# paulvoliva/XNODE-WAN-PDE-solver

Measured on AMD Instinct MI355X. Metric: WAN training-steps/sec (optimiser sub-steps, d=20 cube, N_r=4096 paths per GPU), higher is better.
Workload: dtype f64

## Files before the change

xnode_wan_pde_solver_amd/_lib.py:

```python
import ctypes
import os

_HERE = os.path.dirname(os.path.abspath(__file__))
LIB_PATH = os.environ.get('XW_LIBRARY') or os.path.join(_HERE, 'libxnwan.so')
ABI_VERSION = 33

c_f32p = ctypes.c_void_p
c_f64p = ctypes.c_void_p
c_i64p = ctypes.c_void_p
c_int, c_dbl, c_vp = ctypes.c_int, ctypes.c_double, ctypes.c_void_p


class XwOdeFwdJob(ctypes.Structure):
    _fields_ = [('xT', c_vp), ('start', c_vp), ('u', c_vp), ('Y', c_vp), ('act', c_vp), ('N', c_int), ('act_x_only', c_int),
                ('narrow', c_int), ('prio_drop', c_int)]


class XwOdeBwdJob(ctypes.Structure):
    _fields_ = [('xT', c_vp), ('start', c_vp), ('Y', c_vp), ('act', c_vp), ('ubar', c_vp), ('gx', c_vp), ('gs', c_vp),
                ('gslab', c_vp), ('N', c_int), ('res_first_only', c_int), ('res_u', c_vp), ('res_ref', c_vp),
                ('res_coef', ctypes.c_double), ('res_base', ctypes.c_double), ('res_w_per_point', c_int), ('res_w', c_vp),
                ('res_c', c_vp), ('res_cp', c_vp), ('res_kappa2', ctypes.c_double), ('res_scal', c_vp), ('res_refA', c_vp),
                ('res_coefA', ctypes.c_double), ('res_baseA', ctypes.c_double)]

# ... 52 lines not shown
    'xw_ode_act_rows': [c_int, c_int, c_int, c_int],
    'xw_ode_bwd_multi': [ctypes.POINTER(XwOdeBwdJob), c_int, c_f32p, c_f64p, c_int, c_int, c_int, c_int, c_int, c_int, c_int, c_vp],
    'xw_tiled_ode_ok': [c_int, c_int, c_int, c_int],
    'xw_tiled_ode_work': [c_int, c_int, c_int, c_int, c_int],
    'xw_tiled_ode_bwd_slabs': [c_int],
    'xw_tiled_ode_fwd_multi': [ctypes.POINTER(XwOdeFwdJob), c_int, c_f32p, c_f64p, c_int, c_int, c_int, c_int, c_int, c_int, c_f64p,
                               c_f64p, c_vp],
    'xw_tiled_ode_bwd_multi': [ctypes.POINTER(XwOdeBwdJob), c_int, c_f32p, c_f64p, c_int, c_int, c_int, c_int, c_int, c_int, c_int,
                               c_f64p, c_vp],
    'xw_paths_tiled_work': [c_int, c_int, c_int, c_int],
    'xw_paths_tiled_fwd': [ctypes.POINTER(XwPathsJob), c_int, c_f64p, c_int, c_int, c_int, c_int, c_int, c_int, c_f64p, c_vp],
    'xw_adams_coef': [c_int, c_vp],
    'xw_adams_tiled_work': [c_int, c_int, c_int, c_int, c_int],
    'xw_adams_tiled_fwd_multi': [ctypes.POINTER(XwOdeFwdJob), c_int, c_f32p, c_f64p, c_int, c_int, c_int, c_int, c_int, c_f64p, c_f64p,
                                 c_vp],
    'xw_adams_tiled_bwd_multi': [ctypes.POINTER(XwOdeBwdJob), c_int, c_f32p, c_f64p, c_int, c_int, c_int, c_int, c_int, c_int, c_f64p,
                                 c_vp],
    'xw_dopri5_ctl_size': [],
    'xw_dopri5_work_size': [c_int],
    'xw_dopri5_init': [ctypes.POINTER(XwDopriJob), c_int, c_f32p, c_f64p, c_int, c_int, c_int, c_int, c_int, c_int, c_dbl, c_dbl,
                       c_vp],
    'xw_dopri5_attempts': [ctypes.POINTER(XwDopriJob), c_int, c_f32p, c_f64p, c_int, c_int, c_int, c_int, c_int, c_int, c_dbl,
                           c_dbl, c_int, c_int, c_vp],
    'xw_dopri5_sweep': [ctypes.POINTER(XwDopriSweepJob), c_int, c_f32p, c_f64p, c_int, c_int, c_int, c_int, c_int, c_int, c_vp],
    'xw_tdopri5_work': [c_int, c_int, c_int, c_int, c_int],
    'xw_tdopri5_part_size': [c_int],
    'xw_tdopri5_init': [ctypes.POINTER(XwDopriJob), c_int, c_f32p, c_f64p, c_int, c_int, c_int, c_int, c_int, c_int, c_dbl, c_dbl,
                        c_f64p, c_vp],
    'xw_tdopri5_attempts': [ctypes.POINTER(XwDopriJob), c_int, c_f32p, c_f64p, c_int, c_int, c_int, c_int, c_int, c_int, c_dbl,
                            c_dbl, c_int, c_int, c_f64p, c_vp],
    'xw_tdopri5_sweep': [ctypes.POINTER(XwDopriSweepJob), c_int, c_f32p, c_f64p, c_int, c_int, c_int, c_int, c_int, c_int, c_f64p,
                         c_vp],
    'xw_ode_bwd': [c_f32p, c_f32p, c_f64p, c_f64p, c_f64p, c_f64p, c_int, c_int, c_int, c_int, c_int, c_int, c_int, c_int,
                   c_f64p, c_f64p, c_f64p, c_vp],
    'xw_disc_fwd': [c_f32p, c_f32p, c_f32p, c_f64p, c_int, c_int, c_int, c_int, c_int, c_f64p, c_f64p, c_f64p, c_f64p, c_int,
                    c_int, c_f64p, c_vp],
    'xw_disc_xproj': [c_f32p, c_f64p, c_int, c_int, c_int, c_f64p, c_vp],
    'xw_disc_fwd_xproj': [c_f32p, c_f32p, c_f32p, c_f64p, c_int, c_int, c_int, c_int, c_int, c_f64p, c_f64p, c_f64p, c_f64p, c_int,
                          c_int, c_f64p, c_f64p, c_vp],
    'xw_disc_act_rows': [c_int, c_int],
    'xw_disc_gradx': [c_f32p, c_f32p, c_f32p, c_f64p, c_f64p, c_int, c_int, c_int, c_int, c_f64p, c_f64p, c_vp],
    'xw_disc_bwd_slabs': [c_int, c_int],
    'xw_disc_bwd': [c_f32p, c_f32p, c_f32p, c_f64p, c_f64p, c_int, c_int, c_int, c_int, c_int, c_f64p, c_f64p, c_vp],
    'xw_disc_tiled_ok': [c_int, c_int, c_int],
    'xw_disc_tiled_act_rows': [c_int, c_int],
    'xw_disc_tiled_fwd': [c_f32p, c_f32p, c_f32p, c_f64p, c_int, c_int, c_int, c_int, c_int, c_f64p, c_f64p, c_f64p, c_f64p, c_int,
                          c_int, c_f64p, c_f64p, c_vp],
    'xw_disc_tiled_bwd': [c_f32p, c_f32p, c_f32p, c_f64p, c_f64p, c_int, c_int, c_int, c_int, c_int, c_f64p, c_f64p, c_vp],
    'xw_mt19937_uniform_f32': [c_vp, ctypes.c_long, c_vp, ctypes.c_long, ctypes.c_float, ctypes.c_float, c_int],
    'xw_gather_fields': [c_vp, c_int, ctypes.c_long, c_vp],
    'xw_mt19937_legacy_normal_f64': [c_vp, ctypes.POINTER(c_int), ctypes.POINTER(c_int), ctypes.POINTER(c_dbl), c_vp, ctypes.c_long],
    'xw_weak_partials': [c_f64p, c_f64p, c_f64p, c_f64p, c_int, c_f64p, c_f64p, c_f64p, c_f64p, c_f64p, c_f64p, c_f64p,
                         c_f64p, c_int, c_f64p, c_dbl, c_f64p, c_f64p, c_f64p, c_int, c_dbl, c_int, c_int, c_dbl, c_dbl, c_f64p, c_f64p,
                         c_int, c_int, c_dbl, c_dbl, c_dbl, c_dbl, c_i64p, c_f64p, c_f64p, ctypes.c_long, c_vp],
    'xw_pair_fold': [c_f64p, c_dbl, c_dbl, c_vp],
    'xw_cube_weight': [c_vp, c_int, c_int, c_dbl, c_dbl, c_f64p, c_f64p, c_f64p, c_f64p, c_vp],
    'xw_bdry_partials': [c_f64p, c_f64p, c_int, c_int, c_dbl, c_dbl, c_f64p, c_f64p, c_f64p, c_vp],
    'xw_reduce_work_size': [],
    'xw_weak_contract_general': [c_f64p, c_int, c_f64p, c_f64p, c_f64p, c_f64p, c_f64p, c_f64p, c_f64p, c_f64p, c_int, c_int, c_f64p, c_vp],
    'xw_gen_cotangents': [c_f64p, c_f64p, c_f64p, c_int, c_f64p, c_f64p, c_dbl, c_f64p, c_int, c_int, c_dbl, c_dbl, c_dbl,
                          c_dbl, c_f64p, c_f64p, c_f64p, c_vp],
    'xw_disc_cotangent': [c_f64p, c_f64p, c_f64p, c_int, c_f64p, c_dbl, c_f64p, c_f64p, c_int, c_int, c_dbl, c_dbl, c_dbl,
                          c_dbl, c_f64p, c_f64p, c_vp],
    'xw_losses': [c_f64p, c_int, c_int, c_dbl, c_dbl, c_dbl, c_dbl, c_dbl, c_dbl, c_i64p, c_vp],
    'xw_adam': [c_f64p, c_f64p, c_int, c_f64p, c_f64p, c_int, c_f64p, c_f64p, c_f64p, c_f64p, c_i64p, c_int, c_int, c_dbl,
                c_dbl, c_dbl, c_dbl, c_f64p, c_int, c_int, c_int, c_i64p, c_vp],
    'xw_substep_gen': [ctypes.POINTER(XwGroup), ctypes.POINTER(XwSolverState), c_int, c_int, c_f64p, c_int, c_vp],
    'xw_substep_disc': [ctypes.POINTER(XwGroup), ctypes.POINTER(XwSolverState), c_int, c_int, c_f64p, c_vp],
    'xw_slab_sum': [c_f64p, c_int, c_int, c_int, c_f64p, c_vp],
    'xw_slab_sum2': [c_f64p, c_int, c_f64p, c_f64p, c_int, c_f64p, c_int, c_vp],
    'xw_comm_available': [],
    'xw_comm_unique_id': [ctypes.c_char_p],
    'xw_comm_init': [ctypes.c_char_p, c_int, c_int, ctypes.POINTER(c_vp)],
    'xw_allreduce': [c_f64p, c_int, c_vp, c_vp],
    'xw_comm_destroy': [c_vp],
}

EVAL_SIGNATURES = {
    'xw_paths_dopri5_work': [c_int, c_int, c_int, c_int],
    'xw_paths_dopri5_fwd': [ctypes.POINTER(XwPathsDopriJob), c_int, c_f64p, c_int, c_int, c_int, c_int, c_int, c_dbl, c_dbl, c_int,
                            c_int, c_f64p, c_vp],
}

ERRORS = {-1: 'XW_E_DIMS: network widths/depths not among the compiled kernel instantiations',
          -2: 'XW_E_ARG: null pointer, non-positive size or bad enum',
          -3: 'XW_E_WORKSPACE: workspace too small',
          -4: 'XW_E_COMM: RCCL is not available in this process, or a collective call failed'}


class XnwanError(RuntimeError):
    pass


def _load():
    if not os.path.exists(LIB_PATH):
        raise XnwanError(
            'libxnwan.so not found at %s -- build it with `python -c "import __graft_entry__ as g; g.build()"` '
            'or `make -C xnode_wan_pde_solver_amd/csrc`.  There is no CPU fallback.' % LIB_PATH)
    import torch
    lib = ctypes.CDLL(LIB_PATH)
    for name, argtypes in list(SIGNATURES.items()) + list(EVAL_SIGNATURES.items()):
        fn = getattr(lib, name)
        fn.argtypes = argtypes
        fn.restype = ctypes.c_int
    got = lib.xw_abi_version()
    if got != ABI_VERSION:
        raise XnwanError('libxnwan.so ABI version %d, host expects %d -- rebuild' % (got, ABI_VERSION))
    return lib


lib = _load()


def check(status, what):
    if status == 0:
        return
    if status in ERRORS:
        buf = ctypes.create_string_buffer(512)
        lib.xw_supported_dims(buf, 512)
        raise XnwanError('%s: %s (compiled: %s)' % (what, ERRORS[status], buf.value.decode()))
    raise XnwanError('%s: HIP launch error %d' % (what, status))
```

xnode_wan_pde_solver_amd/csrc/xw_disc_bwd.hip:

```cpp
#include "xw_disc_core.h"
#include <cstdlib>

namespace {

template <int W> struct BwdLds {
  typedef VDim<W> D;
  static constexpr int nfrag = D::MT * D::KS * 64;
  static constexpr int ntt = 4 * D::MT * XW_TTILE;
  static constexpr int oVh = 0, oVhT = nfrag, oD = 2 * nfrag, oR = 2 * nfrag + ntt, oO = 2 * nfrag + 2 * ntt;
  static constexpr int oB = oO + 4 * 64 * 16;
  static constexpr int total = oB + 2 * 16 * D::MT;
  static_assert(total * 8 <= 160 * 1024, "LDS budget of one CU");
};

template <int W, int Q, int CTG, bool PARAMS, bool INGRAD>
__global__ void __launch_bounds__(256) k_disc_bwd(const double* __restrict__ xT, const double* __restrict__ tf,
                                                  const double* __restrict__ tpp, const double* __restrict__ ph,
                                                  const double* __restrict__ vbar, int N, int L, int d,
                                                  double* __restrict__ gslab, double* __restrict__ gxv,
                                                  double* __restrict__ gtv) {
  typedef VDim<W> D;
  typedef BwdLds<W> S;
  static_assert(D::MT == 4, "the recomputing reverse kernel maps the 4 row tiles of dVh onto the 4 waves of a block");
  static_assert(D::BIASROW, "the recomputing reverse kernel takes dVh.b from the ones row");
  __shared__ double lds[S::total];
  double* sVh = lds + S::oVh;
  double* sVhT = lds + S::oVhT;
  double* sD = lds + S::oD;
  double* sR = lds + S::oR;
  double* sO = lds + S::oO;
  const int lane = xw_lane(), g = lane >> 4, n = lane & 15;
  const int wave = threadIdx.x >> 6;
  const VOff o = v_offsets(d, W);
  const long P = (long)N * L;
  const long nsuper = (P + 63) / 64;

  double* sB = lds + S::oB;
  for (int idx = wave; idx < D::MT * D::KS; idx += 4) {
    const int mt = idx / D::KS, ks = idx - mt * D::KS;
    sVh[idx * 64 + lane] = xw_fragA(ph + o.Vh, W, W, W, 16 * mt, 4 * ks);
    sVhT[idx * 64 + lane] = xw_fragAT(ph + o.Vh, W, W, W, 16 * mt, 4 * ks);
  }
  if (threadIdx.x < 16 * D::MT) {
    sB[threadIdx.x] = (int)threadIdx.x < W ? ph[o.Vhb + threadIdx.x] : 0.0;
    sB[16 * D::MT + threadIdx.x] = (int)threadIdx.x < W ? ph[o.Vo + threadIdx.x] : 0.0;
  }
  if (PARAMS)
    for (int i = 0; i < 16; ++i) sO[i * 256 + wave * 64 + lane] = 0.0;
  __syncthreads();

  d4 accH[D::MT], accIn[CTG * 4];
#pragma unroll
  for (int ct = 0; ct < D::MT; ++ct) accH[ct] = xw_zero4();
#pragma unroll
  for (int ct = 0; ct < CTG * 4; ++ct) accIn[ct] = xw_zero4();

  auto layer = [&](const d4 (&r)[D::MT], d4 (&out)[D::MT]) {
    asm volatile("" ::: "memory");
#pragma unroll
    for (int mt = 0; mt < D::MT; ++mt)
#pragma unroll
      for (int rr = 0; rr < 4; ++rr) out[mt][rr] = sB[16 * mt + g + 4 * rr];
#pragma unroll
    for (int ks = 0; ks < D::KS; ++ks) {
      const double b = r[ks >> 2][ks & 3];
#pragma unroll
      for (int mt = 0; mt < D::MT; ++mt) out[mt] = XW_MFMA(sVh[(mt * D::KS + ks) * 64 + lane], b, out[mt]);
    }
  };

  constexpr int SEG = CTG == 1 ? 1 : 3;
  constexpr int NSEG = (Q + SEG - 1) / SEG;
  for (long st = blockIdx.x; st < nsuper; st += gridDim.x) {
    const Pt pt = locate(st * 4 + wave, P, N, tf, tpp);
    d4 ck[NSEG][D::MT];
    d4 a[D::MT], ad[D::MT];
    input_layer<W>(ph, o, xT, N, d, pt, a, ad);
#pragma unroll
    for (int j = 0; j < Q; ++j) {
      d4 r[D::MT];
#pragma unroll
      for (int mt = 0; mt < D::MT; ++mt) {
#pragma unroll
// ... 122 lines not shown
          vv = XW_MFMA(xw_fragAT(ph + o.Vin + 1, o.ldin, W, d, 16 * rt, 4 * ks), dl[ks >> 2][ks & 3], vv);
#pragma unroll
        for (int r = 0; r < 4; ++r) {
          const int i = 16 * rt + g + 4 * r;
          if (i < d && pt.valid) gxv[(long)i * P + pt.p] = vv[r];
        }
      }
      double st_ = 0.0;
#pragma unroll
      for (int mt = 0; mt < D::MT; ++mt) {
        const d4 v0 = xw_vecD_strided(ph + o.Vin, o.ldin, W, 16 * mt);
#pragma unroll
        for (int r = 0; r < 4; ++r) st_ += v0[r] * dl[mt][r];
      }
      st_ = xw_sum_over_g(st_);
      if (gtv != nullptr && g == 0 && pt.valid) gtv[pt.p] = st_;
    }
  }

  if (PARAMS) {
    double* slab = gslab + (long)blockIdx.x * o.total;
#pragma unroll
    for (int ct = 0; ct < D::MT; ++ct) {
      const int c = 16 * ct + n;
#pragma unroll
      for (int r = 0; r < 4; ++r) {
        const int row = 16 * wave + g + 4 * r;
        if (row < W) {
          if (c < W) slab[o.Vh + row * W + c] = accH[ct][r];
          else if (c == W) slab[o.Vhb + row] = accH[ct][r];
        }
      }
    }
#pragma unroll
    for (int ct = 0; ct < CTG * 4; ++ct) {
      const int c = 16 * ct + n;
#pragma unroll
      for (int r = 0; r < 4; ++r) {
        const int row = 16 * wave + g + 4 * r;
        if (row < W) {
          if (c <= d) slab[o.Vin + row * o.ldin + c] = accIn[ct][r];
          else if (c == d + 1) slab[o.Vinb + row] = accIn[ct][r];
        }
      }
    }
    __syncthreads();
    const int tid = threadIdx.x;
    if (tid <= W) {
      double s = 0.0;
      if (tid < W) {
        const int mt = tid >> 4, gg = tid & 3, r = (tid & 15) >> 2;
        for (int wv = 0; wv < 4; ++wv)
          for (int nn = 0; nn < 16; ++nn) s += sO[(mt * 4 + r) * 256 + wv * 64 + gg * 16 + nn];
        slab[o.Vo + tid] = s;
      } else {
        for (int wv = 0; wv < 4; ++wv)
          for (int nn = 0; nn < 16; ++nn) s += sO[15 * 256 + wv * 64 + nn];
        slab[o.Vob] = s;
      }
    }
  }
}

typedef void (*BwdKernel)(const double*, const double*, const double*, const double*, const double*, int, int, int, double*,
                          double*, double*);
const BwdKernel bwd_table[2][2] = {{k_disc_bwd<50, 9, 1, true, false>, k_disc_bwd<50, 9, 1, false, true>},
                                   {k_disc_bwd<50, 9, 2, true, false>, k_disc_bwd<50, 9, 2, false, true>}};

void launch_recompute(bool ingrad, const double* xT, const double* t, const double* tpp, const double* phi, const double* vbar,
                      int N, int L, int d, double* gslab, double* gxv, double* gtv, void* stream) {
  const int ctg = d + 2 <= 64 ? 1 : 2;
  hipLaunchKernelGGL(bwd_table[ctg - 1][ingrad ? 1 : 0], dim3(bwd_blocks((long)N * L)), dim3(256), 0, (hipStream_t)stream, xT, t,
                     tpp, phi, vbar, N, L, d, gslab, gxv, gtv);
}

struct RecKey {
  int ng;
  bool tsum;
};
RecKey rec_select(int N, int d, bool point_mode, bool tsum_on) {
  return {d + 2 <= 48 ? 1 : d + 2 <= 96 ? 2 : 3, tsum_on && !point_mode && (N % 64) == 0};
}

}

extern "C" int xw_disc_bwd_slabs(int N, int L) { return bwd_blocks((long)N * L); }

extern "C" int xw_disc_bwd(const double* xT, const double* t, const double* tpp, const double* phi, const double* vbar,
                           int N, int L, int d, int W, int q, const double* act, double* gslab, void* stream) {
  if (!xT || !phi || !gslab || N <= 0 || L <= 0 || d <= 0) return XW_E_ARG;
  if (!tpp && !t) return XW_E_ARG;
  if (tpp && L != 1) return XW_E_ARG;
  if (!disc_width_ok(W)) return xwg_disc_bwd(xT, t, tpp, phi, vbar, N, L, d, W, q, act, gslab, bwd_blocks((long)N * L), stream);
  if (q < 0 || d + 2 > 128 || ((q != 9 || W != 50) && act == nullptr)) return XW_E_DIMS;
  if ((long)N * L * 4 >= (1L << 31)) return XW_E_ARG;
  if (act != nullptr) {
    static const bool tsum_on = [] { const char* e = getenv("XW_DISC_REC_TSUM"); return !(e && e[0] == '0'); }();
    const RecKey k = rec_select(N, d, tpp != nullptr, tsum_on);
    return xw_disc_rec_launch(W, k.ng, k.tsum, bwd_blocks((long)N * L), xT, t, tpp, phi, vbar, N, L, d, gslab, act, q, stream);
  }
  launch_recompute(false, xT, t, tpp, phi, vbar, N, L, d, gslab, nullptr, nullptr, stream);
  return xw_launch_status();
}

extern "C" int xw_disc_gradx(const double* xT, const double* t, const double* tpp, const double* phi, const double* vbar,
                             int N, int d, int W, int q, double* gxv, double* gtv, void* stream) {
  if (!xT || !phi || !gxv || N <= 0 || d <= 0) return XW_E_ARG;
  if (!tpp && !t) return XW_E_ARG;
  if (W != 50 || q != 9 || d + 2 > 128) return XW_E_DIMS;
  launch_recompute(true, xT, t, tpp, phi, vbar, N, 1, d, nullptr, gxv, gtv, stream);
  return xw_launch_status();
}
```

xnode_wan_pde_solver_amd/csrc/xw_disc_core.h:

```cpp
#pragma once
#include "xw_common.h"
#include "xw_generic.h"

namespace {

template <int W> struct VDim {
  static constexpr int MT = (W + 15) / 16;
  static constexpr int KS = (W + 3) / 4;
  static constexpr int TR = W - 16 * (MT - 1);
  static constexpr bool VTAIL = TR <= 3;
  static constexpr int MTF = VTAIL ? MT - 1 : MT;
  __device__ static constexpr int LR(int mt) { return (W + 1 - 16 * mt) >= 16 ? 4 : (W + 1 - 16 * mt + 3) / 4; }
  static constexpr bool BIASROW = (W % 16) != 0;
  static_assert(MT == 4 || MT == 6 || MT == 8, "row tiles of the compiled widths");
};

struct Pt {
  int p, n;
  bool valid;
  double t;
};
__device__ __forceinline__ Pt locate(long tile, long P, int N, const double* __restrict__ tf, const double* __restrict__ tpp) {
  Pt q;
  const long p = tile * 16 + (xw_lane() & 15);
  q.valid = p < P;
  const long pc = q.valid ? p : P - 1;
  q.p = (int)pc;
  if (tpp != nullptr) {
    q.n = (int)pc;
    q.t = tpp[pc];
  } else {
    const int l = (int)(pc / N);
    q.n = (int)(pc - (long)l * N);
    q.t = tf[l];
  }
  return q;
}

template <int W>
__device__ __forceinline__ void input_layer(const double* __restrict__ ph, const VOff& o, const double* __restrict__ xT,
                                            int N, int d, const Pt& q, d4 (&a)[VDim<W>::MT], d4 (&ad)[VDim<W>::MT]) {
  typedef VDim<W> D;
  const int g = xw_lane() >> 4;
#pragma unroll
  for (int mt = 0; mt < D::MT; ++mt) {
    ad[mt] = xw_vecD_strided(ph + o.Vin, o.ldin, W, 16 * mt);
    a[mt] = xw_vecD(ph + o.Vinb, W, 16 * mt) + ad[mt] * q.t;
  }
  for (int ks = 0; ks < (d + 3) / 4; ++ks) {
    const int i = 4 * ks + g;
    const double b = i < d ? xT[(long)i * N + q.n] : 0.0;
#pragma unroll
    for (int mt = 0; mt < D::MT; ++mt) a[mt] = XW_MFMA(xw_fragA(ph + o.Vin + 1, o.ldin, W, d, 16 * mt, 4 * ks), b, a[mt]);
  }
}

#define XW_QMAX 16

inline bool disc_width_ok(int W) { return W == 50 || W == 64 || W == 96 || W == 128; }

inline int bwd_blocks(long P) {
  long nsuper = (P + 63) / 64;
  return (int)(nsuper < 512 ? nsuper : 512);
}

}

XWG_HIDDEN int xw_disc_rec_launch(int W, int ng, bool tsum, int blocks, const double* xT, const double* t, const double* tpp,
                                  const double* phi, const double* vbar, int N, int L, int d, double* gslab, const double* act,
                                  int q, void* stream);
```

xnode_wan_pde_solver_amd/csrc/xw_disc_rec.hip:

```cpp
#include "xw_disc_core.h"

namespace {

#ifdef XW_REC_PROBE
__device__ unsigned long long xw_rec_clock[12 * 2048];
#define XW_PH(i) { const unsigned long long t_ = __builtin_amdgcn_s_memtime(); phc[i] += t_ - phl; phl = t_; }
#else
#define XW_PH(i)
#endif
template <int W> struct RecLds {
  typedef VDim<W> D;
  static constexpr bool VT = D::VTAIL;
  static_assert(!VT || D::LR(D::MT - 1) == 1, "short last row tile: vector-ALU tail + one live 4-row group");
  static constexpr int T3 = VT ? 4 * XW_TSTRIDE : XW_TTILE;
  static constexpr int wset = (D::MT - 1) * XW_TTILE + T3;
  static constexpr bool FRAG_LDS = D::MT == 4;
  static constexpr int oVhT = 0;
  static constexpr int oTT = oVhT + (FRAG_LDS ? D::MTF * D::KS * 64 : 0);
  static constexpr int oVo = oTT + (VT ? 4 * D::KS * D::TR : 0);
  static constexpr int oD = oVo + 16 * D::MT;
  static constexpr int oR = oD + 4 * wset;
  static constexpr int oO = oR + 4 * wset;
  static constexpr int NO = 4 * D::MT;
  static constexpr int total = oO + (NO + 1) * 16;
  static_assert(total * 8 <= (VT ? 80 : 160) * 1024, "two blocks per CU (short tail) / one");
  __device__ static constexpr int toff(int mt) { return mt * XW_TTILE; }
};

template <int W> __device__ __forceinline__ double rec_readT(const double* set, int mt, int ks) {
  const int l = xw_lane();
  const int row = (RecLds<W>::VT && mt == VDim<W>::MT - 1) ? (l & 3) : (l & 15);
  return set[RecLds<W>::toff(mt) + row * XW_TSTRIDE + 4 * ks + (l >> 4)];
}

template <int W, int Q, int NG, bool TSUM>
__global__ void __launch_bounds__(256, RecLds<W>::VT ? 2 : 1) k_disc_rec(const double* __restrict__ xT, const double* __restrict__ tf,
                                                     const double* __restrict__ tpp, const double* __restrict__ ph,
                                                     const double* __restrict__ vbar, int N, int L, int d,
                                                     double* __restrict__ gslab, const double* __restrict__ act, int qrt) {
  typedef VDim<W> D;
  typedef RecLds<W> S;
  __shared__ double lds[S::total];
  double* sVhT = lds + S::oVhT;
  double* sTT = lds + S::oTT;
  double* sVo = lds + S::oVo;
  double* sO = lds + S::oO;
  const int lane = xw_lane(), g = lane >> 4, n = lane & 15;
  const int wave = threadIdx.x >> 6;
  double* myD = lds + S::oD + wave * S::wset;
  double* myR = lds + S::oR + wave * S::wset;
#ifdef XW_REC_PROBE
  const unsigned long long ck_in = __builtin_amdgcn_s_memtime(), rt_in = __builtin_amdgcn_s_memrealtime();
#endif
  const VOff o = v_offsets(d, W);
  const long P = (long)N * L;
  const long nsuper = (P + 63) / 64;
  const int nq = Q > 0 ? Q : qrt;
  constexpr int UNROLL = Q > 0 ? Q : 1;
  constexpr int TW = D::MT / 2;
  const int wi = wave >> 1, wj = wave & 1;

  if (S::FRAG_LDS)
    for (int idx = wave; idx < D::MTF * D::KS; idx += 4) {
      const int mt = idx / D::KS, ks = idx - mt * D::KS;
      sVhT[idx * 64 + lane] = xw_fragAT(ph + o.Vh, W, W, W, 16 * mt, 4 * ks);
    }
  if (S::VT)
    for (int idx = threadIdx.x; idx < 4 * D::KS * D::TR; idx += blockDim.x) {
      const int r = idx % D::TR, k = idx / D::TR;
      sTT[idx] = k < W ? ph[o.Vh + (long)k * W + 16 * (D::MT - 1) + r] : 0.0;
    }
  if (threadIdx.x < 16 * D::MT) sVo[threadIdx.x] = (int)threadIdx.x < W ? ph[o.Vo + threadIdx.x] : 0.0;
  for (int idx = threadIdx.x; idx < (S::NO + 1) * 16; idx += blockDim.x) sO[idx] = 0.0;
  __syncthreads();

  d4 accH[TW * TW], accB[D::MT];
#pragma unroll
  for (int ct = 0; ct < TW * TW; ++ct) accH[ct] = xw_zero4();
#pragma unroll
  for (int ct = 0; ct < D::MT; ++ct) accB[ct] = xw_zero4();
  constexpr bool EDGE = S::VT;
  constexpr int NE = 7;
  double accE[NE];
#pragma unroll
  for (int e = 0; e < NE; ++e) accE[e] = 0.0;
  const int vstart = wave == 1 ? 7 : wave == 3 ? 6 : 0;
  const int lane16 = (lane & 15) * XW_TSTRIDE + (lane >> 4);
  const int lane4 = (lane & 3) * XW_TSTRIDE + ((lane >> 2) & 3) * 4 + (lane >> 4);
  const int offC = (wave < 3 ? S::oD + wave * XW_TTILE : S::oR + 2 * XW_TTILE) + lane16;
  const int offW = (wave < 3 ? S::oR : S::oD) + lane16;
  const int offX = (wave < 2 ? S::oD : S::oR) + 48 * XW_TSTRIDE + lane4;
  const int offV = (wave < 2 ? S::oR : S::oD) + vstart * 4 * XW_TSTRIDE + lane4;
  double* slab = gslab + (long)blockIdx.x * o.total;

#ifdef XW_REC_PROBE
  unsigned long long phc[8] = {0, 0, 0, 0, 0, 0, 0, 0}, phl = __builtin_amdgcn_s_memtime();
#endif
  const long ngs = N >> 6;
  const long ub = nsuper / gridDim.x, ur = nsuper % gridDim.x;
  const long u0 = (long)blockIdx.x * ub + ((long)blockIdx.x < ur ? (long)blockIdx.x : ur), u1 = u0 + ub + ((long)blockIdx.x < ur ? 1 : 0);
  d4 sumS[D::MT], sumT[D::MT];
#pragma unroll
  for (int mt = 0; mt < D::MT; ++mt) sumS[mt] = sumT[mt] = xw_zero4();
  bool slab_first = true;
  for (long it = TSUM ? u0 : (long)blockIdx.x; it < (TSUM ? u1 : nsuper); it += TSUM ? 1 : (long)gridDim.x) {
    const long ung = TSUM ? it / L : 0;
    const long st = TSUM ? (it - ung * L) * ngs + ung : it;
    const Pt pt = locate(st * 4 + wave, P, N, tf, tpp);
    const long ntile = (P + 15) >> 4;
    const long tl = st * 4 + wave < ntile ? st * 4 + wave : ntile - 1;
    const double* tbase = act + (long)__builtin_amdgcn_readfirstlane((int)tl) * ((long)(nq + 1) * W * 16);
    const int aoff = lane;
    auto load_layer = [&](int j, d4 (&r)[D::MT]) {
      const double* base = tbase + j * W * 16;
      asm volatile("" : "+s"(base));
#pragma unroll
      for (int mt = 0; mt < D::MT; ++mt)
#pragma unroll
        for (int q_ = 0; q_ < 4; ++q_)
          if (q_ < D::LR(mt)) {
            const int row = 16 * mt + 4 * q_ + g;
            r[mt][q_] = (16 * mt + 4 * q_ + 3 < W || row < W) ? xw_ld_nt(base + (16 * mt + 4 * q_) * 16 + aoff) : 0.0;
          }
    };
    d4 a[D::MT], rnext[D::MT];
    load_layer(nq, a);
    if (nq > 0) load_layer(nq - 1, rnext);
    const double vb = pt.valid ? (vbar != nullptr ? xw_ld_g(vbar + pt.p) : 1.0) : 0.0;
    d4 dl[D::MT];
#pragma unroll
    for (int mt = 0; mt < D::MT; ++mt)
#pragma unroll
      for (int r = 0; r < 4; ++r) {
        if (r < D::LR(mt) && 16 * mt + 4 * r < W) {
          const double th = a[mt][r];
          dl[mt][r] = sVo[16 * mt + g + 4 * r] * (1.0 - th * th) * vb;
          const double s_ = xw_sum_over_n(vb * th);
          if (n == 0) sO[(mt * 4 + r) * 16 + wave * 4 + g] += s_;
        } else {
          dl[mt][r] = 0.0;
        }
      }
    {
      const double s_ = xw_sum_over_n(vb);
      if (lane == 0) sO[S::NO * 16 + wave * 4] += s_;
    }
    XW_PH(6)
#pragma unroll UNROLL
    for (int sg = nq - 1; sg >= 0; --sg) {
      bool open[4 * D::MT];
#pragma unroll
      for (int mt = 0; mt < D::MT; ++mt)
#pragma unroll
        for (int r = 0; r < 4; ++r) open[4 * mt + r] = r < D::LR(mt) && rnext[mt][r] > 0.0;
#pragma unroll
      for (int mt = 0; mt < D::MT; ++mt) {
        d4 rr = rnext[mt];
        if (D::BIASROW && mt == (W >> 4)) {
          if (g == ((W & 15) & 3)) rr[(W & 15) >> 2] = 1.0;
        }
        if (!D::BIASROW) accB[mt] = accB[mt] + dl[mt];
        if (mt < D::MT - 1 || !S::VT) {
          xw_writeT(myD + S::toff(mt), dl[mt]);
          xw_writeT(myR + S::toff(mt), rr);
        } else {
          xw_writeT_n<1>(myD + S::toff(mt), dl[mt]);
          xw_writeT_n<1>(myR + S::toff(mt), rr);
        }
      }
      if (sg > 0) load_layer(sg - 1, rnext);
      XW_PH(0)
      d4 nd[D::MT];
      asm volatile("" ::: "memory");
#pragma unroll
      for (int mt = 0; mt < D::MT; ++mt) nd[mt] = xw_zero4();
      double tv[D::TR];
#pragma unroll
      for (int r = 0; r < D::TR; ++r) tv[r] = 0.0;
      if constexpr (S::FRAG_LDS) {
#pragma unroll
        for (int ks = 0; ks < D::KS; ++ks) {
          const double b = dl[ks >> 2][ks & 3];
          if ((ks & 1) == 0) asm volatile("" ::: "memory");
#pragma unroll
          for (int mt = 0; mt < D::MTF; ++mt) nd[mt] = XW_MFMA(sVhT[(mt * D::KS + ks) * 64 + lane], b, nd[mt]);
          if (S::VT) {
#pragma unroll
            for (int r = 0; r < D::TR; ++r) tv[r] = fma(sTT[(4 * ks + g) * D::TR + r], b, tv[r]);
          }
        }
      } else {
        const double* phg = ph;
        int ll = lane;
        asm volatile("" : "+s"(phg), "+v"(ll));
        double fn[D::MT];
#pragma unroll
        for (int mt = 0; mt < D::MT; ++mt) fn[mt] = xw_fragAT_l(phg + o.Vh, W, W, W, 16 * mt, 0, ll);
#pragma unroll
        for (int ks = 0; ks < D::KS; ++ks) {
          const double b = dl[ks >> 2][ks & 3];
          double fc[D::MT];
#pragma unroll
          for (int mt = 0; mt < D::MT; ++mt) fc[mt] = fn[mt];
          if (ks + 1 < D::KS) {
#pragma unroll
            for (int mt = 0; mt < D::MT; ++mt) fn[mt] = xw_fragAT_l(phg + o.Vh, W, W, W, 16 * mt, 4 * (ks + 1), ll);
          }
          asm volatile("" ::: "memory");
#pragma unroll
          for (int mt = 0; mt < D::MT; ++mt) nd[mt] = XW_MFMA(fc[mt], b, nd[mt]);
        }
// ... 174 lines not shown
#pragma unroll
    for (int t2 = 0; t2 < 2; ++t2)
#pragma unroll
      for (int r = 0; r < 4; ++r) {
        const int row = wave < 3 ? 16 * wave + g + 4 * r : 16 * t2 + n, c = wave < 3 ? 16 * t2 + n : 32 + g + 4 * r;
        slab[o.Vh + row * W + c] = accH[t2][r];
      }
    __syncthreads();
    double* s22 = lds + S::oD;
#pragma unroll
    for (int r = 0; r < 4; ++r) s22[wave * 256 + (g + 4 * r) * 16 + n] = accH[2][r];
    __syncthreads();
    {
      const int i = threadIdx.x >> 4, j = threadIdx.x & 15;
      slab[o.Vh + (32 + i) * W + 32 + j] = (s22[threadIdx.x] + s22[256 + threadIdx.x]) + (s22[512 + threadIdx.x] + s22[768 + threadIdx.x]);
    }
#pragma unroll
    for (int e = 0; e < NE; ++e) {
      double s_ = accE[e];
      s_ += __shfl_xor(s_, 4);
      s_ += __shfl_xor(s_, 8);
      if ((e < NE - 1 || wave == 0) && (lane & 12) == 0) {
        const int i = lane >> 4, j = lane & 3, blk = vstart + e;
        const int row = wave < 2 ? 48 + i : 4 * blk + j, c = wave < 2 ? 4 * blk + j : 48 + i;
        if (row < W) {
          if (c < W) slab[o.Vh + row * W + c] = s_;
          else if (c == W) slab[o.Vhb + row] = s_;
        }
      }
    }
  } else {
#pragma unroll
    for (int t4 = 0; t4 < TW * TW; ++t4) {
      const int c = 16 * (TW * wj + (t4 % TW)) + n;
#pragma unroll
      for (int r = 0; r < 4; ++r) {
        const int row = 16 * (TW * wi + (t4 / TW)) + g + 4 * r;
        if (row < W) {
          if (c < W) slab[o.Vh + row * W + c] = accH[t4][r];
          else if (c == W) slab[o.Vhb + row] = accH[t4][r];
        }
      }
    }
  }
  __syncthreads();
  const int tid = threadIdx.x;
  if (!D::BIASROW) {
    double* sBsum = lds + S::oD;
#pragma unroll
    for (int mt = 0; mt < D::MT; ++mt)
#pragma unroll
      for (int r = 0; r < 4; ++r) {
        const double s_ = xw_sum_over_n(accB[mt][r]);
        if (n == 0) sBsum[wave * 16 * D::MT + 16 * mt + 4 * r + g] = s_;
      }
    __syncthreads();
    if (tid < W) slab[o.Vhb + tid] = sBsum[tid] + sBsum[16 * D::MT + tid] + sBsum[32 * D::MT + tid] + sBsum[48 * D::MT + tid];
  }
  if (tid <= W) {
    double s_ = 0.0;
    if (tid < W) {
      const int mt = tid >> 4, gg = tid & 3, r = (tid & 15) >> 2;
      for (int wv = 0; wv < 4; ++wv) s_ += sO[(mt * 4 + r) * 16 + wv * 4 + gg];
      slab[o.Vo + tid] = s_;
    } else {
      for (int wv = 0; wv < 4; ++wv) s_ += sO[S::NO * 16 + wv * 4];
      slab[o.Vob] = s_;
    }
  }
#ifdef XW_REC_PROBE
  if (lane == 0 && blockIdx.x * 4 + wave < 2048) {
    unsigned long long* o_ = xw_rec_clock + 12 * (blockIdx.x * 4 + wave);
    for (int i = 0; i < 8; ++i) o_[i] = phc[i];
    const unsigned long long ck_out = __builtin_amdgcn_s_memtime();
    o_[8] = ck_loop - ck_in - (phc[0] + phc[1] + phc[2] + phc[3] + phc[4] + phc[5] + phc[6] + phc[7]);
    o_[9] = ck_out - ck_loop;
    o_[10] = ck_out - ck_in;
    o_[11] = __builtin_amdgcn_s_memrealtime() - rt_in;
  }
#endif
}

typedef void (*RecKernel)(const double*, const double*, const double*, const double*, const double*, int, int, int, double*,
                          const double*, int);
struct RecRow {
  int W;
  RecKernel k[3][2];
};
template <int W> constexpr RecRow rec_row() {
  return {W, {{k_disc_rec<W, 0, 1, false>, k_disc_rec<W, 0, 1, true>},
              {k_disc_rec<W, 0, 2, false>, k_disc_rec<W, 0, 2, true>},
              {k_disc_rec<W, 0, 3, false>, k_disc_rec<W, 0, 3, true>}}};
}
const RecRow rec_table[] = {rec_row<50>(), rec_row<64>(), rec_row<96>(), rec_row<128>()};

}

int xw_disc_rec_launch(int W, int ng, bool tsum, int blocks, const double* xT, const double* t, const double* tpp,
                       const double* phi, const double* vbar, int N, int L, int d, double* gslab, const double* act, int q,
                       void* stream) {
  if (ng < 1 || ng > 3) return XW_E_DIMS;
  for (const RecRow& row : rec_table)
    if (row.W == W) {
      hipLaunchKernelGGL(row.k[ng - 1][tsum ? 1 : 0], dim3(blocks), dim3(256), 0, (hipStream_t)stream, xT, t, tpp, phi, vbar, N, L,
                         d, gslab, act, q);
      return xw_launch_status();
    }
  return XW_E_DIMS;
}

#ifdef XW_REC_PROBE
extern "C" int xw_debug_rec_clock(unsigned long long* host, int nwaves) {
  return (int)hipMemcpyFromSymbol(host, HIP_SYMBOL(xw_rec_clock), sizeof(unsigned long long) * 12 * nwaves);
}
#endif
```

xnode_wan_pde_solver_amd/csrc/xw_substep.hip:

```cpp
#include <hip/hip_runtime.h>
#include <string.h>
#include "xnwan.h"

namespace {
struct Side {
  hipStream_t s = nullptr;
  hipEvent_t fork = nullptr, fwd = nullptr, done = nullptr;
};
Side* side_of_current_device() {
  static Side sides[64];
  int dev = 0;
  if (hipGetDevice(&dev) != hipSuccess || dev < 0 || dev >= 64) return nullptr;
  Side& x = sides[dev];
  if (x.s == nullptr) {
    if (hipStreamCreateWithFlags(&x.s, hipStreamNonBlocking) != hipSuccess) return nullptr;
    if (hipEventCreateWithFlags(&x.fork, hipEventDisableTiming) != hipSuccess || hipEventCreateWithFlags(&x.fwd, hipEventDisableTiming) != hipSuccess ||
        hipEventCreateWithFlags(&x.done, hipEventDisableTiming) != hipSuccess)
      return nullptr;
  }
  return &x;
}
#define XW_HIP(call) { const hipError_t e_ = (call); if (e_ != hipSuccess) return (int)e_; }

inline XwOdeFwdJob fwd_job(const double* xT, const double* start, double* u, double* Y, double* act, int N, int x_only, int narrow) {
  XwOdeFwdJob j;
  j.xT = xT; j.start = start; j.u = u; j.Y = Y; j.act = act; j.N = N; j.act_x_only = x_only; j.narrow = narrow; j.prio_drop = 0;
  return j;
}
inline XwOdeBwdJob bwd_job(const double* xT, const double* start, const double* Y, const double* act, int N) {
  XwOdeBwdJob j;
  memset(&j, 0, sizeof(j));
  j.xT = xT; j.start = start; j.Y = Y; j.act = act; j.N = N;
  return j;
}
#define XW_TRY(call) { const int rc_ = (call); if (rc_ != 0) return rc_; }

int test_net(const XwGroup* g, const XwSolverState* s, int blocks, double* record, void* stream) {
  if (g->tpp != nullptr)
    return xw_disc_fwd(g->xvT_pts, nullptr, g->tpp, s->phi, g->N * g->L, 1, g->d, s->W, s->q, g->v, g->vt, g->gxv, g->gtv, g->N, blocks,
                       record, stream);
  if (g->xproj != nullptr && g->xproj_current != 2) XW_TRY(xw_disc_xproj(g->xvT, s->phi, g->N, g->d, s->W, g->xproj, stream));
  return xw_disc_fwd_xproj(g->xvT, g->t, nullptr, s->phi, g->N, g->L, g->d, s->W, s->q, g->v, g->vt, g->gxv, g->gtv, g->N, blocks, record,
                           g->xproj, stream);
}
int contract(const XwGroup* g, const XwSolverState* s, long long* step, bool with_bdry, bool finalize, void* stream) {
  const double* s3x = nullptr;
  if (g->A0 != nullptr || g->B0 != nullptr) {
    XW_TRY(xw_weak_contract_general(g->A0, g->amode, g->B0, g->gx, g->gs, g->ghT, g->gxv, g->w0, g->gwx0T, g->v, g->d, g->N, g->s3x,
                                    stream));
    s3x = g->s3x;
  }
  const bool fused = s3x == nullptr;
  return xw_weak_partials(g->u, g->v, g->vt, g->w, g->w_per_point, g->wt, s3x, fused ? g->gx : nullptr, fused ? g->gs : nullptr,
                          fused ? g->ghT : nullptr, fused ? g->gxv : nullptr, fused ? g->w0 : nullptr, fused ? g->gwx0T : nullptr,
                          fused ? g->d : 0, g->c, g->ckappa, g->f, g->h, g->pair_i ? g->href : nullptr, g->pair_i ? 1 : 0,
                          g->pair_i ? g->s3_scale : 1.0, g->N, g->L, g->Vol, g->Nglob, g->work_i, s->scal, finalize ? 1 : 0,
                          g->Lb > 0 ? g->Lb : 1, g->Nbglob, s->alpha, g->init_off, g->bdry_off, finalize ? step : nullptr, with_bdry && g->Nb > 0 ? g->ub : nullptr,
                          with_bdry && g->Nb > 0 ? g->g : nullptr, with_bdry && g->Nb > 0 ? (long)g->Nb * g->Lb : 0, stream);
}
inline bool sharded(const XwGroup* g, const XwSolverState* s) { return g->sharded != 0 && s->exchange != nullptr; }
#define XW_ZERO(ptr, count) XW_HIP(hipMemsetAsync((ptr), 0, sizeof(double) * (size_t)(count), (hipStream_t)stream))
}

extern "C" int xw_substep_gen(const XwGroup* g, const XwSolverState* s, int skip_v, int store_record, double* accum,
                              int adam_skip_field, void* stream) {
  if (!g || !s || g->N < 0 || g->Nb < 0 || g->L <= 0) return XW_E_ARG;
  const bool shard = sharded(g, s);
  if (g->N == 0 && !shard) return XW_E_ARG;
  if (shard && (!s->pack_u || s->scal != s->pack_u + 2 * (long)s->Pu)) return XW_E_ARG;
  const bool fused_x = s->pollution == 1.0 && !s->adjoint;
  const bool have_i = g->N > 0, have_b = g->Nb > 0;
  const bool joint = have_i && have_b && g->same_grid;
  const int adj = s->adjoint ? 8 : 0;
  void* const main_stream = stream;
  const bool merged = s->merged_sweep && !shard && accum == nullptr && fused_x && joint && !g->pair_i && !g->pair_b && g->A0 == nullptr &&
                      g->B0 == nullptr;
  if (merged) {
    Side* sd = side_of_current_device();
    if (sd == nullptr) return XW_E_ARG;
    XW_HIP(hipEventRecord(sd->fork, (hipStream_t)main_stream));
    XW_HIP(hipStreamWaitEvent(sd->s, sd->fork, 0));
    if (!skip_v) XW_TRY(test_net(g, s, s->v_blocks, store_record ? g->vact : nullptr, main_stream));
    {
      XwOdeFwdJob jobs[2] = {fwd_job(g->xT, g->start, g->u, g->Y, g->act, g->N, 0, (g->narrow >> 0) & 1),
                             fwd_job(g->xbT, g->start_b, g->ub, g->Yb, g->act_b, g->Nb, 0, (g->narrow >> 0) & 1)};
      XW_TRY(xw_ode_fwd_multi(jobs, 2, g->t, s->theta, s->method, g->L, g->d, s->H, s->K, s->m, s->scal, (void*)sd->s));
      XwOdeBwdJob jx = bwd_job(g->xT, g->start, g->Y, g->act, g->N);
      jx.gx = g->gx; jx.gs = g->gs;
      XW_TRY(xw_ode_bwd_multi(&jx, 1, g->t, s->theta, s->method, g->L, g->d, s->H, s->K, s->m, 1 | (((g->narrow >> 5) & 1) ? 16 : 0),
                              (void*)sd->s));
    }
    XW_HIP(hipEventRecord(sd->fwd, sd->s));
    XW_HIP(hipStreamWaitEvent((hipStream_t)main_stream, sd->fwd, 0));
    XW_TRY(contract(g, s, s->step_u, true, true, main_stream));
    XwOdeBwdJob jobs[2];
    jobs[0] = bwd_job(g->xT, g->start, g->Y, g->act, g->N);
    jobs[0].gslab = g->slabA;
    jobs[0].res_first_only = 3; jobs[0].res_u = g->u; jobs[0].res_ref = g->v;
    jobs[0].res_coef = g->Vol / g->Nglob / g->L * g->s3_scale; jobs[0].res_base = g->Vol / g->Nglob;
    jobs[0].res_w_per_point = g->w_per_point; jobs[0].res_w = g->w; jobs[0].res_c = g->c; jobs[0].res_cp = g->cp;
    jobs[0].res_kappa2 = 2.0 * g->ckappa;
    jobs[0].res_scal = s->scal; jobs[0].res_refA = g->h; jobs[0].res_coefA = 2.0 * s->alpha / g->Nglob; jobs[0].res_baseA = s->pollution;
    jobs[1] = bwd_job(g->xbT, g->start_b, g->Yb, g->act_b, g->Nb);
    jobs[1].gslab = g->slabA + (long)g->ns_u * s->Pu;
    jobs[1].res_u = g->ub; jobs[1].res_ref = g->g; jobs[1].res_first_only = 0;
    jobs[1].res_coef = 2.0 * s->alpha / (g->Nbglob * g->Lb); jobs[1].res_base = 0.0;
    XW_TRY(xw_ode_bwd_multi(jobs, 2, g->t, s->theta, s->method, g->L, g->d, s->H, s->K, s->m, 2 | (((g->narrow >> 4) & 1) ? 16 : 0),
                            main_stream));
    return xw_adam(s->theta, g->slabA, g->ns_u + g->ns_b, nullptr, nullptr, 0, nullptr, nullptr, s->m_u, s->v_u, s->step_u, -1, s->Pu,
                   s->lr_u, s->beta1, s->beta2, s->eps, s->grad_u, s->lag_lo, s->lag_hi, adam_skip_field, s->lag_u, main_stream);
  }
  if (have_i) {
    Side* sd = side_of_current_device();
    if (sd == nullptr) return XW_E_ARG;
    XW_HIP(hipEventRecord(sd->fork, (hipStream_t)main_stream));
    XW_HIP(hipStreamWaitEvent(sd->s, sd->fork, 0));
    if (!skip_v) XW_TRY(test_net(g, s, s->v_blocks, store_record ? g->vact : nullptr, main_stream));
    stream = (void*)sd->s;
    {
      XwOdeFwdJob jobs[2] = {fwd_job(g->xT, g->start, g->u, g->Y, g->act, g->N, 0, (g->narrow >> 0) & 1),
                             fwd_job(g->xbT, g->start_b, g->ub, g->Yb, g->act_b, g->Nb, 0, (g->narrow >> 0) & 1)};
      XW_TRY(xw_ode_fwd_multi(jobs, joint ? 2 : 1, g->t, s->theta, s->method, g->L, g->d, s->H, s->K, s->m, s->scal, stream));
      if (have_b && !joint) {
        XwOdeFwdJob jb = fwd_job(g->xbT, g->start_b, g->ub, g->Yb, g->act_b, g->Nb, 0, (g->narrow >> 1) & 1);
        XW_TRY(xw_ode_fwd_multi(&jb, 1, g->tb, s->theta, s->method, g->Lb, g->d, s->H, s->K, s->m, nullptr, stream));
      }
    }
    XW_HIP(hipEventRecord(sd->fwd, sd->s));
    stream = main_stream;
    XW_HIP(hipStreamWaitEvent((hipStream_t)main_stream, sd->fwd, 0));
  } else {
    XW_ZERO(s->scal, 16);
    if (have_b) {
      XwOdeFwdJob jb = fwd_job(g->xbT, g->start_b, g->ub, g->Yb, g->act_b, g->Nb, 0, (g->narrow >> 1) & 1);
      XW_TRY(xw_ode_fwd_multi(&jb, 1, g->tb, s->theta, s->method, g->Lb, g->d, s->H, s->K, s->m, nullptr, stream));
    }
  }
  if (have_i && !fused_x) {
    XwOdeBwdJob jx = bwd_job(g->xT, g->start, g->Y, g->act, g->N);
    jx.gx = g->gx; jx.gs = g->gs;
    XW_TRY(xw_ode_bwd_multi(&jx, 1, g->t, s->theta, s->method, g->L, g->d, s->H, s->K, s->m, 1 | adj | (((g->narrow >> 5) & 1) ? 16 : 0),
                            stream));
  }
  {
    XwOdeBwdJob jobs[3];
    int nj = 0;
    if (have_i) {
      jobs[nj] = bwd_job(g->xT, g->start, g->Y, g->act, g->N);
      jobs[nj].gslab = g->slabA;
      if (fused_x) { jobs[nj].gx = g->gx; jobs[nj].gs = g->gs; }
      jobs[nj].res_u = g->u; jobs[nj].res_ref = g->pair_i ? g->href : g->h; jobs[nj].res_first_only = 1;
      jobs[nj].res_coef = 2.0 * s->alpha / g->Nglob; jobs[nj].res_base = s->pollution;
      ++nj;
    }
    XwOdeBwdJob jb = bwd_job(g->xbT, g->start_b, g->Yb, g->act_b, g->Nb);
    if (have_b) {
      jb.gslab = g->slabA + (long)g->ns_u * s->Pu;
      jb.res_u = g->ub; jb.res_ref = g->g; jb.res_first_only = 0;
      jb.res_coef = 2.0 * s->alpha / (g->Nbglob * g->Lb); jb.res_base = 0.0;
    }
    if (joint) jobs[nj++] = jb;
    if (have_i) {
      XwOdeBwdJob jB = bwd_job(g->xT, g->start, g->Y, g->act, g->N);
      jB.gslab = g->slabB;
      jB.res_first_only = 2; jB.res_u = g->u; jB.res_ref = g->v;
      jB.res_coef = g->Vol / g->Nglob / g->L * g->s3_scale; jB.res_base = g->Vol / g->Nglob;
      jB.res_w_per_point = g->w_per_point; jB.res_w = g->w; jB.res_c = g->c; jB.res_cp = g->cp; jB.res_kappa2 = 2.0 * g->ckappa;
      jobs[nj++] = jB;
      const int modeA = (fused_x ? (1 | 2 | 4) : 2) | adj | (((g->narrow >> 2) & 1) ? 16 : 0);
      XW_TRY(xw_ode_bwd_multi(jobs, nj, g->t, s->theta, s->method, g->L, g->d, s->H, s->K, s->m, modeA, stream));
    }
    if (have_b && !joint)
      XW_TRY(xw_ode_bwd_multi(&jb, 1, g->tb, s->theta, s->method, g->Lb, g->d, s->H, s->K, s->m, 2 | adj | (((g->narrow >> 3) & 1) ? 16 : 0),
                              stream));
  }
  if (have_i) {
    XW_TRY(contract(g, s, s->step_u, true, !shard, stream));
  } else if (have_b) {
    XW_TRY(xw_bdry_partials(g->ub, g->g, g->Nb, g->Lb, s->alpha, g->Nbglob, nullptr, g->work_b, s->scal, stream));
  }
  if (!shard) {
    XW_TRY(xw_adam(s->theta, g->slabA, g->ns_u + g->ns_b, accum, g->slabB, g->ns_u, nullptr, s->scal, s->m_u, s->v_u, s->step_u, -1, s->Pu,
                   s->lr_u, s->beta1, s->beta2, s->eps, s->grad_u, s->lag_lo, s->lag_hi, adam_skip_field, s->lag_u, stream));
  } else {
    const int nA = (have_i ? g->ns_u : 0) + (have_b ? g->ns_b : 0), nB = have_i ? g->ns_u : 0;
    double* const pA = s->pack_u;
    double* const pB = s->pack_u + s->Pu;
    if (nA > 0 && nB > 0) {
      XW_TRY(xw_slab_sum2(g->slabA, nA, pA, g->slabB, nB, pB, s->Pu, stream));
    } else {
      if (nA > 0) { XW_TRY(xw_slab_sum(g->slabA + (have_i ? 0 : (long)g->ns_u * s->Pu), nA, s->Pu, 0, pA, stream)); } else { XW_ZERO(pA, s->Pu); }
      XW_ZERO(pB, s->Pu);
    }
    XW_TRY(s->exchange(s->pack_u, 2 * s->Pu + 16, s->exchange_ctx, stream));
    if (g->pair_i) XW_TRY(xw_pair_fold(s->scal, g->Vol, g->Nglob, stream));
    XW_TRY(xw_losses(s->scal, g->L, g->Lb > 0 ? g->Lb : 1, g->Vol, g->Nglob, g->Nbglob, s->alpha, g->init_off, g->bdry_off, s->step_u, stream));
    XW_TRY(xw_adam(s->theta, accum, accum != nullptr ? 1 : 0, pA, nullptr, 0, pB, s->scal, s->m_u, s->v_u, s->step_u, -1, s->Pu, s->lr_u,
                   s->beta1, s->beta2, s->eps, s->grad_u, s->lag_lo, s->lag_hi, adam_skip_field, s->lag_u, stream));
  }
  if (accum != nullptr) {
    const hipError_t e = hipMemcpyAsync(accum, s->grad_u, sizeof(double) * s->Pu, hipMemcpyDeviceToDevice, (hipStream_t)stream);
    if (e != hipSuccess) return (int)e;
  }
  return 0;
}

extern "C" int xw_substep_disc(const XwGroup* g, const XwSolverState* s, int skip_v, int use_record, double* accum, void* stream) {
  if (!g || !s || g->N < 0 || g->L <= 0) return XW_E_ARG;
  const bool shard = sharded(g, s);
  if (g->N == 0 && !shard) return XW_E_ARG;
  const bool have_i = g->N > 0;
  const int adj = s->adjoint ? 8 : 0;
  double* record = use_record ? g->vact : nullptr;
  void* const main_stream = stream;
  if (have_i) {
    Side* sd = side_of_current_device();
    if (sd == nullptr) return XW_E_ARG;
    XW_HIP(hipEventRecord(sd->fork, (hipStream_t)main_stream));
    XW_HIP(hipStreamWaitEvent(sd->s, sd->fork, 0));
    if (!skip_v) XW_TRY(test_net(g, s, s->v_blocks_disc, record, main_stream));
    stream = (void*)sd->s;
    {
      XwOdeFwdJob jf = fwd_job(g->xT, g->start, g->u, g->Y, g->act, g->N, 1, (g->narrow >> 6) & 1);
      XW_TRY(xw_ode_fwd_multi(&jf, 1, g->t, s->theta, s->method, g->L, g->d, s->H, s->K, s->m, s->scal, stream));
      XwOdeBwdJob jx = bwd_job(g->xT, g->start, g->Y, g->act, g->N);
      jx.gx = g->gx; jx.gs = g->gs;
      XW_TRY(xw_ode_bwd_multi(&jx, 1, g->t, s->theta, s->method, g->L, g->d, s->H, s->K, s->m, 1 | adj | (((g->narrow >> 7) & 1) ? 16 : 0),
                              stream));
    }
    XW_HIP(hipEventRecord(sd->done, sd->s));
    stream = main_stream;
    XW_HIP(hipStreamWaitEvent((hipStream_t)main_stream, sd->done, 0));
    XW_TRY(contract(g, s, s->step_v, false, !shard, stream));
  } else {
    XW_ZERO(s->scal, 16);
  }
  if (shard) {
    XW_TRY(s->exchange(s->scal, 9, s->exchange_ctx, stream));
    if (g->pair_i) XW_TRY(xw_pair_fold(s->scal, g->Vol, g->Nglob, stream));
  }
  const int nsv = have_i ? xw_disc_bwd_slabs(g->N, g->L) : 0;
  if (have_i) {
    XW_TRY(xw_disc_cotangent(g->u, g->v, g->w, g->w_per_point, g->c, g->ckappa, g->f, g->h, g->N, g->L, g->Vol, g->Nglob, s->pollution,
                             g->s3_scale, s->scal, g->vbar, stream));
    if (g->tpp != nullptr) {
      XW_TRY(xw_disc_bwd(g->xvT_pts, nullptr, g->tpp, s->phi, g->vbar, g->N * g->L, 1, g->d, s->W, s->q, record, g->slab_v, stream));
    } else {
      XW_TRY(xw_disc_bwd(g->xvT, g->t, nullptr, s->phi, g->vbar, g->N, g->L, g->d, s->W, s->q, record, g->slab_v, stream));
    }
  }
  if (!shard) {
    XW_TRY(xw_adam(s->phi, g->slab_v, nsv, accum, nullptr, 0, nullptr, nullptr, s->m_v, s->v_v, s->step_v, -1, s->Pv, s->lr_v, s->beta1,
                   s->beta2, s->eps, s->grad_v, 0, 0, 0, nullptr, stream));
  } else {
    if (have_i) { XW_TRY(xw_slab_sum(g->slab_v, nsv, s->Pv, 0, s->grad_v, stream)); } else { XW_ZERO(s->grad_v, s->Pv); }
    XW_TRY(s->exchange(s->grad_v, s->Pv, s->exchange_ctx, stream));
    XW_TRY(xw_losses(s->scal, g->L, g->Lb > 0 ? g->Lb : 1, g->Vol, g->Nglob, g->Nbglob, s->alpha, 0.0, 0.0, s->step_v, stream));
    XW_TRY(xw_adam(s->phi, accum, accum != nullptr ? 1 : 0, s->grad_v, nullptr, 0, nullptr, nullptr, s->m_v, s->v_v, s->step_v, -1, s->Pv,
                   s->lr_v, s->beta1, s->beta2, s->eps, s->grad_v, 0, 0, 0, nullptr, stream));
  }
  if (have_i && g->xproj != nullptr && g->tpp == nullptr && g->xproj_current != 0 && accum == nullptr)
    XW_TRY(xw_disc_xproj(g->xvT, s->phi, g->N, g->d, s->W, g->xproj, stream));
  if (accum != nullptr) {
    const hipError_t e = hipMemcpyAsync(accum, s->grad_v, sizeof(double) * s->Pv, hipMemcpyDeviceToDevice, (hipStream_t)stream);
    if (e != hipSuccess) return (int)e;
  }
  return 0;
}
```

xnode_wan_pde_solver_amd/csrc/xw_weak.hip:

```cpp
#include "xw_common.h"
#include "xnwan.h"

namespace {

__device__ __forceinline__ double wave_sum(double x) { return xw_sum_over_g(xw_sum_over_n(x)); }
#define XW_REDUCE_TICKET (6 * 1024)
template <int NV>
__device__ __forceinline__ bool grid_sum(double (&val)[NV], double* __restrict__ work, double* __restrict__ dst) {
  __shared__ double red[NV][16];
  __shared__ int is_last;
  const int wave = threadIdx.x >> 6, lane = threadIdx.x & 63;
#pragma unroll
  for (int i = 0; i < NV; ++i) {
    const double s = wave_sum(val[i]);
    if (lane == 0) red[i][wave] = s;
  }
  __syncthreads();
  if (threadIdx.x < NV) {
    double s = 0.0;
    for (int w = 0; w < (int)(blockDim.x >> 6); ++w) s += red[threadIdx.x][w];
    work[(long)blockIdx.x * NV + threadIdx.x] = s;
  }
  asm volatile("s_waitcnt vmcnt(0)" ::: "memory");
  __syncthreads();
  unsigned int* ticket = reinterpret_cast<unsigned int*>(work + XW_REDUCE_TICKET);
  if (threadIdx.x == 0) {
    __builtin_amdgcn_fence(__ATOMIC_RELEASE, "agent");
    asm volatile("s_waitcnt vmcnt(0)" ::: "memory");
    const unsigned int t = __hip_atomic_fetch_add(ticket, 1u, __ATOMIC_RELAXED, __HIP_MEMORY_SCOPE_AGENT);
    is_last = (t == gridDim.x - 1);
    if (is_last) {
      __builtin_amdgcn_fence(__ATOMIC_ACQUIRE, "agent");
      asm volatile("s_waitcnt vmcnt(0)" ::: "memory");
    }
  }
  __syncthreads();
  if (!is_last) return false;
#pragma unroll
  for (int i = 0; i < NV; ++i) {
    double part = 0.0;
    for (unsigned int b = threadIdx.x; b < gridDim.x; b += blockDim.x) part += work[(long)b * NV + i];
    const double s = wave_sum(part);
    if (lane == 0) red[i][wave] = s;
  }
  __syncthreads();
  if (threadIdx.x < NV) {
    double tot = 0.0;
    for (int w = 0; w < (int)(blockDim.x >> 6); ++w) tot += red[threadIdx.x][w];
    dst[threadIdx.x < 3 ? threadIdx.x : (threadIdx.x < 5 ? threadIdx.x + 4 : threadIdx.x - 2)] += tot;
  }
  if (threadIdx.x == 0) *ticket = 0u;
  return true;
}

__device__ __forceinline__ double interior_loss(const double* scal, double Vol, double Nglob, int L) {
  const double I = scal[0], S = scal[1];
  return log(I * I) - log(Vol * S / (Nglob * (double)L));
}

__device__ __forceinline__ void fold_pairs(double* scal, double cN) {
  scal[0] -= cN * scal[7] * scal[8];
  scal[7] = 0.0;
  scal[8] = 0.0;
}
__device__ __forceinline__ void loss_values(double* scal, int L, int Lb, double Vol, double Nglob, double Nbglob,
                                            double alpha, double init_off, double bdry_off) {
  const double in_ = interior_loss(scal, Vol, Nglob, L);
  scal[6] = in_;
  scal[4] = in_ + alpha * ((scal[2] / Nglob + init_off) + (scal[3] / (Nbglob * (double)Lb) + bdry_off));
  scal[5] = -in_;
}

__global__ void __launch_bounds__(1024) k_weak_partials(const double* __restrict__ u, const double* __restrict__ v,
                                                       const double* __restrict__ vt, const double* __restrict__ w,
                                                       int w_per_point, const double* __restrict__ wt,
                                                       const double* __restrict__ s3x, const double* __restrict__ gx,
                                                       const double* __restrict__ gs, const double* __restrict__ ghT,
                                                       const double* __restrict__ gxv, const double* __restrict__ w0,
                                                       const double* __restrict__ gwx0T, int d,
                                                       const double* __restrict__ c, double ckappa,
                                                       const double* __restrict__ f, const double* __restrict__ h,
                                                       const double* __restrict__ href, int pairwise, double s3_scale,
                                                       int N, int L, double Vol, double Nglob, double* __restrict__ work,
                                                       double* __restrict__ scal, int finalize, int Lb, double Nbglob,
                                                       double alpha, double init_off, double bdry_off,
                                                       long long* __restrict__ step, const double* __restrict__ ub,
                                                       const double* __restrict__ gb, long Pb) {
  double acc[6] = {0.0, 0.0, 0.0, 0.0, 0.0, 0.0};
  const double cN = Vol / Nglob, cNL = Vol / Nglob / (double)L;
  const long P = (long)N * L;
  for (long p = (long)blockIdx.x * blockDim.x + threadIdx.x; p < P; p += (long)gridDim.x * blockDim.x) {
    const int l = (int)(p / N), n = (int)(p - (long)l * N);
    const double ul = u[p], vl = v[p];
    const double wl = w_per_point ? w[p] : w[n];
    const double phi = vl * wl;
    double phit = wl * vt[p];
    if (wt != nullptr) phit += vl * wt[p];
    const double cl = c != nullptr ? c[p] : ckappa * ul;
    double s3 = cl * ul * phi + f[p] * phi;
    double I = 0.0;
    if (l == 0) {
      const double hn = h[n];
      double s31;
      s31 = s3x != nullptr ? s3x[n] : 0.0;
      s3 += s31;
      I -= cN * hn * vl;
      const double hr = href != nullptr ? href[n] : hn;
      acc[2] += (ul - hr) * (ul - hr);
    }
    if (s3x == nullptr) {
      double part = 0.0;
      if (l < d) {
        const double w0n = w0[n], gsn = gs[n], v0n = v[n];
        for (int i = l; i < d; i += L) {
          const long q = (long)i * N + n;
          part += (w0n * gxv[q] + v0n * gwx0T[q]) * (gx[q] + gsn * ghT[q]);
        }
      }
      I += cNL * s3_scale * part;
    }
    if (l == L - 1) I += cN * ul * vl;
    if (pairwise) {
      I += cNL * s3_scale * s3;
      acc[3] += ul;
      acc[4] += phit;
    } else {
      I -= cNL * (ul * phit - s3_scale * s3);
    }
    acc[0] += I;
    acc[1] += vl * vl;
  }
  if (ub != nullptr)
    for (long p = (long)blockIdx.x * blockDim.x + threadIdx.x; p < Pb; p += (long)gridDim.x * blockDim.x) {
      const double r = ub[p] - gb[p];
      acc[5] += r * r;
    }
  const bool last = grid_sum<6>(acc, work, scal);
  if (finalize && last) {
    __syncthreads();
    if (threadIdx.x == 0) {
      if (step != nullptr) *step += 1;
      if (pairwise) fold_pairs(scal, cN);
      loss_values(scal, L, Lb, Vol, Nglob, Nbglob, alpha, init_off, bdry_off);
    }
  }
}

__global__ void __launch_bounds__(1024) k_bdry(const double* __restrict__ ub, const double* __restrict__ gb, long P,
                                              double coef, double* __restrict__ ubar_b, double* __restrict__ work,
                                              double* __restrict__ scal) {
  double acc[1] = {0.0};
  for (long p = (long)blockIdx.x * blockDim.x + threadIdx.x; p < P; p += (long)gridDim.x * blockDim.x) {
    const double r = ub[p] - gb[p];
    acc[0] += r * r;
    if (ubar_b != nullptr) ubar_b[p] = coef * r;
  }
  grid_sum<1>(acc, work, scal + 3);
}


__global__ void __launch_bounds__(256) k_gen_cots(const double* __restrict__ u, const double* __restrict__ v,
                                                  const double* __restrict__ w, int w_per_point,
                                                  const double* __restrict__ c, const double* __restrict__ cp,
                                                  double ckappa, const double* __restrict__ h, int N, int L, double Vol,
                                                  double Nglob, double alpha, double pollution,
                                                  const double* __restrict__ scal, double* __restrict__ ubarA,
                                                  double* __restrict__ ubarB) {
  const double cI = scal != nullptr ? 2.0 / scal[0] : 0.0;
  const double cN = Vol / Nglob, cNL = Vol / Nglob / (double)L;
  const long P = (long)N * L;
  for (long p = (long)blockIdx.x * blockDim.x + threadIdx.x; p < P; p += (long)gridDim.x * blockDim.x) {
    const int l = (int)(p / N), n = (int)(p - (long)l * N);
    const double ul = u[p];
    const bool needB = ubarB != nullptr || scal != nullptr;
    const double vl = needB ? v[p] : 0.0;
    const double wl = w_per_point ? w[p] : w[n];
    const double dcu = c != nullptr ? c[p] + ul * cp[p] : 2.0 * ckappa * ul;
    double gB = 0.0;
    if (needB) {
      gB = cNL * dcu * vl * wl;
      if (l == L - 1) gB += cN * vl;
      if (ubarB != nullptr) ubarB[p] = gB;
    }
    if (ubarA != nullptr) {
      double gA = pollution;
      if (l == 0) gA += alpha * 2.0 * (ul - h[n]) / Nglob;
      ubarA[p] = gA + cI * gB;
    }
  }
}

__global__ void k_losses(double* __restrict__ scal, int L, int Lb, double Vol, double Nglob, double Nbglob, double alpha,
                         double init_off, double bdry_off, long long* __restrict__ step) {
  if (blockIdx.x == 0 && threadIdx.x == 0) {
    if (step != nullptr) *step += 1;
    loss_values(scal, L, Lb, Vol, Nglob, Nbglob, alpha, init_off, bdry_off);
  }
}
__global__ void k_pair_fold(double* __restrict__ scal, double cN) {
  if (blockIdx.x == 0 && threadIdx.x == 0) fold_pairs(scal, cN);
}

__global__ void __launch_bounds__(256) k_cube_weight(const float* __restrict__ x, int N, int d, float top, float bot,
                                                     double* __restrict__ w, double* __restrict__ w0,
                                                     double* __restrict__ gwT, double* __restrict__ xT) {
  for (int n = blockIdx.x * blockDim.x + threadIdx.x; n < N; n += gridDim.x * blockDim.x) {
    const float* xn = x + (long)n * d;
    float at = fabsf(top - xn[0]), ab = fabsf(bot - xn[0]);
    int it = 0, ib = 0;
    for (int i = 1; i < d; ++i) {
      const float a = fabsf(top - xn[i]), b = fabsf(bot - xn[i]);
      if (a < at) { at = a; it = i; }
      if (b < ab) { ab = b; ib = i; }
    }
    const float wv = ab < at ? ab : at;
    const float ct = (at < ab ? 1.0f : 0.0f) + (at == ab ? 0.5f : 0.0f), cb = (ab < at ? 1.0f : 0.0f) + (at == ab ? 0.5f : 0.0f);
    const float dt = top - xn[it], db = bot - xn[ib];
    const float gt = -(dt > 0.0f ? 1.0f : (dt < 0.0f ? -1.0f : 0.0f)) * ct, gb = -(db > 0.0f ? 1.0f : (db < 0.0f ? -1.0f : 0.0f)) * cb;
    w[n] = (double)wv;
    if (w0) w0[n] = (double)wv;
    for (int i = 0; i < d; ++i) {
      float g = 0.0f;
      if (i == it) g += gt;
      if (i == ib) g += gb;
      gwT[(long)i * N + n] = (double)g;
      if (xT) xT[(long)i * N + n] = (double)xn[i];
    }
  }
}

__global__ void __launch_bounds__(256) k_disc_cot(const double* __restrict__ u, const double* __restrict__ v,
                                                  const double* __restrict__ w, int w_per_point,
                                                  const double* __restrict__ c, double ckappa,
                                                  const double* __restrict__ f, const double* __restrict__ h, int N,
                                                  int L, double Vol, double Nglob, double pollution, double s3_scale,
                                                  const double* __restrict__ scal_in, double* __restrict__ vbar) {
  const double I = scal_in[0], S = scal_in[1];
  const double cI = 2.0 / I;
  const double cN = Vol / Nglob, cNL = Vol / Nglob / (double)L;
  const long P = (long)N * L;
  for (long p = (long)blockIdx.x * blockDim.x + threadIdx.x; p < P; p += (long)gridDim.x * blockDim.x) {
    const int l = (int)(p / N), n = (int)(p - (long)l * N);
    const double ul = u[p], vl = v[p];
    const double wl = w_per_point ? w[p] : w[n];
    const double cl = c != nullptr ? c[p] : ckappa * ul;
    double dI = cNL * s3_scale * (cl * ul + f[p]) * wl;
    if (l == L - 1) dI += cN * ul;
    if (l == 0) dI -= cN * h[n];
    vbar[p] = pollution * wl - cI * dI + 2.0 * vl / S;
  }
}

#define XW_ADAM_PARAMS 16
#define XW_ADAM_GROUPS 64
__global__ void __launch_bounds__(1024) k_adam(double* __restrict__ param, const double* __restrict__ gA, int nA,
                                               const double* eA, const double* __restrict__ gB, int nB,
                                               const double* eB, const double* __restrict__ scal,
                                               double* __restrict__ m, double* __restrict__ v,
                                               const long long* __restrict__ step, int step_is_current, int P, double lr,
                                               double beta1, double beta2, double eps, double* gsum_out,
                                               int lag_lo, int lag_hi, int skip, const long long* __restrict__ lag) {
  __shared__ double red[2][XW_ADAM_GROUPS][XW_ADAM_PARAMS];
  const int tx = threadIdx.x % XW_ADAM_PARAMS, ty = threadIdx.x / XW_ADAM_PARAMS;
  const int i = blockIdx.x * XW_ADAM_PARAMS + tx;
  double a = 0.0, b = 0.0;
  if (i < P) {
    for (int s = ty; s < nA; s += XW_ADAM_GROUPS) a += gA[(long)s * P + i];
    for (int s = ty; s < nB; s += XW_ADAM_GROUPS) b += gB[(long)s * P + i];
  }
  red[0][ty][tx] = a;
  red[1][ty][tx] = b;
  __syncthreads();
  if (ty != 0 || i >= P) return;
  a = eA != nullptr ? eA[i] : 0.0;
  b = eB != nullptr ? eB[i] : 0.0;
#pragma unroll 8
  for (int k = 0; k < XW_ADAM_GROUPS; ++k) {
    a += red[0][k][tx];
    b += red[1][k][tx];
  }
  const double coefB = scal != nullptr ? 2.0 / scal[0] : 1.0;
  const double g = a + coefB * b;
  if (gsum_out != nullptr) gsum_out[i] = g;
  const bool lagged = i >= lag_lo && i < lag_hi;
  if (lagged && skip) return;
  const long long t = *step + (step_is_current ? 0 : 1) - (lagged && lag != nullptr ? *lag : 0);
  const double bc1 = 1.0 - pow(beta1, (double)t), bc2 = 1.0 - pow(beta2, (double)t);
  const double mi = beta1 * m[i] + (1.0 - beta1) * g;
  const double vi = beta2 * v[i] + (1.0 - beta2) * g * g;
  m[i] = mi;
  v[i] = vi;
  param[i] -= (lr / bc1) * (mi / (sqrt(vi) / sqrt(bc2) + eps));
}
__global__ void k_step_inc(long long* step) { *step += 1; }

__global__ void __launch_bounds__(1024) k_slab_sum(const double* __restrict__ gslab, int nslab, int P, int accumulate,
                                                   double* __restrict__ out) {
  __shared__ double red[XW_ADAM_GROUPS][XW_ADAM_PARAMS];
  const int tx = threadIdx.x % XW_ADAM_PARAMS, ty = threadIdx.x / XW_ADAM_PARAMS;
  const int i = blockIdx.x * XW_ADAM_PARAMS + tx;
  double a = 0.0;
  if (i < P)
    for (int s = ty; s < nslab; s += XW_ADAM_GROUPS) a += gslab[(long)s * P + i];
  red[ty][tx] = a;
  __syncthreads();
  if (ty != 0 || i >= P) return;
  double g = accumulate ? out[i] : 0.0;
#pragma unroll 8
  for (int k = 0; k < XW_ADAM_GROUPS; ++k) g += red[k][tx];
  out[i] = g;
}

inline int reduce_cap(long points) {
  static const int v = [] { const char* e = getenv("XW_REDUCE_BLOCKS"); const int x = e ? atoi(e) : 0; return x > 0 && x <= 1024 ? x : 0; }();
  return v ? v : (points > (1L << 18) ? 256 : 128);
}
inline int reduce_threads() {
  static const int v = [] { const char* e = getenv("XW_REDUCE_THREADS"); const int x = e ? atoi(e) : 0; return (x == 256 || x == 512) ? x : 1024; }();
  return v;
}
inline int blocks_for(long n, int per, int cap) {
  long b = (n + per - 1) / per;
  if (b < 1) b = 1;
  return (int)(b > cap ? cap : b);
}


__global__ void __launch_bounds__(256) k_weak_contract(const double* __restrict__ A0, int amode,
                                                       const double* __restrict__ B0, const double* __restrict__ gx,
                                                       const double* __restrict__ gs, const double* __restrict__ ghT,
                                                       const double* __restrict__ gxv, const double* __restrict__ w0,
                                                       const double* __restrict__ gwx0T, const double* __restrict__ v0,
                                                       int d, int N, double* __restrict__ s3x) {
  const int n = blockIdx.x * blockDim.x + threadIdx.x;
  if (n >= N) return;
  const double w = w0[n], v = v0[n], gsn = gs[n];
  double acc = 0.0, bsum = 0.0;
  for (int i = 0; i < d; ++i) {
    const double dphi = w * gxv[(long)i * N + n] + v * gwx0T[(long)i * N + n];
    const double dui = gx[(long)i * N + n] + gsn * ghT[(long)i * N + n];
    if (B0 != nullptr) bsum += B0[(long)i * N + n] * dui;
    if (amode == 0) {
      acc += dphi * dui;
    } else if (amode == 2) {
      acc += A0[(long)i * N + n] * dphi * dui;
    } else {
      double row = 0.0;
      for (int j = 0; j < d; ++j) {
        const double duj = gx[(long)j * N + n] + gsn * ghT[(long)j * N + n];
        const double a = amode == 1 ? A0[i * d + j] : A0[((long)i * d + j) * N + n];
        row += a * duj;
      }
      acc += dphi * row;
    }
  }
  s3x[n] = acc + v * w * bsum;
}
}

extern "C" int xw_weak_partials(const double* u, const double* v, const double* vt, const double* w, int w_per_point,
                                const double* wt, const double* s3x, const double* gx, const double* gs, const double* ghT,
                                const double* gxv, const double* w0, const double* gwx0T, int d, const double* c,
                                double ckappa, const double* f, const double* h, const double* href, int pairwise,
                                double s3_scale, int N, int L, double Vol, double Nglob, double* work, double* scal,
                                int finalize, int Lb, double Nbglob, double alpha, double init_off, double bdry_off,
                                long long* step, const double* ub, const double* gb, long Pb, void* stream) {
  if (!u || !v || !vt || !w || !f || !h || !work || !scal || N <= 0 || L <= 0 || (finalize && Lb <= 0)) return XW_E_ARG;
  if ((ub == nullptr) != (gb == nullptr) || (ub != nullptr && Pb <= 0)) return XW_E_ARG;
  if (!s3x && (!gx || !gs || !ghT || !gxv || !w0 || !gwx0T || d <= 0)) return XW_E_ARG;
  if (pairwise && L != 1) return XW_E_ARG;
  hipLaunchKernelGGL(k_weak_partials, dim3(blocks_for((long)N * L, reduce_threads(), reduce_cap((long)N * L))), dim3(reduce_threads()), 0, (hipStream_t)stream, u, v, vt, w,
                     w_per_point, wt, s3x, gx, gs, ghT, gxv, w0, gwx0T, d, c, ckappa, f, h, href, pairwise, s3_scale, N, L, Vol,
                     Nglob, work, scal, finalize, Lb, Nbglob, alpha, init_off, bdry_off, step, ub, gb, Pb);
  return xw_launch_status();
}

extern "C" int xw_bdry_partials(const double* ub, const double* g, int Nb, int L, double alpha, double Nbglob,
                                double* ubar_b, double* work, double* scal, void* stream) {
  if (!ub || !g || !work || !scal || Nb <= 0 || L <= 0) return XW_E_ARG;
  const long P = (long)Nb * L;
  const double coef = alpha * 2.0 / (Nbglob * (double)L);
  hipLaunchKernelGGL(k_bdry, dim3(blocks_for(P, reduce_threads(), reduce_cap(P))), dim3(reduce_threads()), 0, (hipStream_t)stream, ub, g, P, coef, ubar_b, work, scal);
  return xw_launch_status();
}

extern "C" int xw_gen_cotangents(const double* u, const double* v, const double* w, int w_per_point, const double* c,
                                 const double* cp, double ckappa, const double* h, int N, int L, double Vol, double Nglob,
                                 double alpha, double pollution, const double* scal, double* ubarA, double* ubarB,
                                 void* stream) {
  if (!u || !w || !h || (!ubarA && !ubarB) || ((ubarB || scal) && !v) || (scal && (!ubarA || ubarB)) || N <= 0 || L <= 0)
    return XW_E_ARG;
  if ((c == nullptr) != (cp == nullptr)) return XW_E_ARG;
  hipLaunchKernelGGL(k_gen_cots, dim3(blocks_for((long)N * L, 256, 2048)), dim3(256), 0, (hipStream_t)stream, u, v, w,
                     w_per_point, c, cp, ckappa, h, N, L, Vol, Nglob, alpha, pollution, scal, ubarA, ubarB);
  return xw_launch_status();
}

extern "C" int xw_losses(double* scal, int L, int Lb, double Vol, double Nglob, double Nbglob, double alpha,
                         double init_off, double bdry_off, long long* step, void* stream) {
  if (!scal || L <= 0 || Lb <= 0) return XW_E_ARG;
  hipLaunchKernelGGL(k_losses, dim3(1), dim3(64), 0, (hipStream_t)stream, scal, L, Lb, Vol, Nglob, Nbglob, alpha, init_off,
                     bdry_off, step);
  return xw_launch_status();
}

extern "C" int xw_pair_fold(double* scal, double Vol, double Nglob, void* stream) {
  if (!scal || Nglob <= 0) return XW_E_ARG;
  hipLaunchKernelGGL(k_pair_fold, dim3(1), dim3(64), 0, (hipStream_t)stream, scal, Vol / Nglob);
  return xw_launch_status();
}

extern "C" int xw_cube_weight(const float* x, int N, int d, double top, double bot, double* w, double* w0, double* gwT,
                              double* xT, void* stream) {
  if (!x || !w || !gwT || N <= 0 || d <= 0 || !(top > bot)) return XW_E_ARG;
  hipLaunchKernelGGL(k_cube_weight, dim3(blocks_for(N, 256, 1024)), dim3(256), 0, (hipStream_t)stream, x, N, d, (float)top,
                     (float)bot, w, w0, gwT, xT);
  return xw_launch_status();
}

namespace {
__global__ __launch_bounds__(256) void k_gather_fields(const XwGather* __restrict__ tab, int count, long total) {
  __shared__ long first[1025];
  for (int r = threadIdx.x; r <= count; r += blockDim.x) first[r] = r < count ? tab[r].before : total;
  __syncthreads();
  const long stride = (long)gridDim.x * blockDim.x;
  for (long e = (long)blockIdx.x * blockDim.x + threadIdx.x; e < total; e += stride) {
    int lo = 0, hi = count;
    while (hi - lo > 1) {
      const int mid = (lo + hi) >> 1;
      if (first[mid] <= e) lo = mid; else hi = mid;
    }
    const XwGather g = tab[lo];
    const long local = e - g.before;
    const long k = local % g.n2, ij = local / g.n2, j = ij % g.n1, i = ij / g.n1;
    g.dst[local] = g.src[i * g.s0 + j * g.s1 + k * g.s2];
  }
}
}

extern "C" int xw_gather_fields(const XwGather* table_dev, int count, long total, void* stream) {
  if (!table_dev || count <= 0 || count > 1024 || total <= 0) return XW_E_ARG;
  hipLaunchKernelGGL(k_gather_fields, dim3(blocks_for(total, 256, 2048)), dim3(256), 0, (hipStream_t)stream, table_dev, count, total);
  return xw_launch_status();
}

extern "C" int xw_disc_cotangent(const double* u, const double* v, const double* w, int w_per_point, const double* c,
                                 double ckappa, const double* f, const double* h, int N, int L, double Vol, double Nglob,
                                 double pollution, double s3_scale, const double* scal_in, double* vbar, void* stream) {
  if (!u || !v || !w || !f || !h || !scal_in || !vbar || N <= 0 || L <= 0) return XW_E_ARG;
  hipLaunchKernelGGL(k_disc_cot, dim3(blocks_for((long)N * L, 256, 2048)), dim3(256), 0, (hipStream_t)stream, u, v, w,
                     w_per_point, c, ckappa, f, h, N, L, Vol, Nglob, pollution, s3_scale, scal_in, vbar);
  return xw_launch_status();
}

extern "C" int xw_adam(double* param, const double* gslabA, int nA, const double* gextraA, const double* gslabB, int nB,
                       const double* gextraB, const double* scal, double* m, double* v, long long* step, int bump_step,
                       int P, double lr, double beta1, double beta2, double eps, double* gsum_out, int lag_lo, int lag_hi,
                       int skip, long long* lag, void* stream) {
  if (!param || !m || !v || !step || P <= 0 || nA < 0 || nB < 0 || (nA > 0 && !gslabA) || (nB > 0 && !gslabB)) return XW_E_ARG;
  if (lag_lo < 0 || lag_hi > P || (skip && (!lag || lag_hi <= lag_lo))) return XW_E_ARG;
  hipLaunchKernelGGL(k_adam, dim3((P + XW_ADAM_PARAMS - 1) / XW_ADAM_PARAMS), dim3(1024), 0, (hipStream_t)stream, param, gslabA, nA, gextraA, gslabB,
                     nB, gextraB, scal, m, v, step, bump_step < 0 ? 1 : 0, P, lr, beta1, beta2, eps, gsum_out, lag_lo, lag_hi, skip,
                     lag);
  if (skip) hipLaunchKernelGGL(k_step_inc, dim3(1), dim3(1), 0, (hipStream_t)stream, lag);
  if (bump_step > 0) hipLaunchKernelGGL(k_step_inc, dim3(1), dim3(1), 0, (hipStream_t)stream, step);
  return xw_launch_status();
}

namespace {
__global__ void __launch_bounds__(1024) k_slab_sum2(const double* __restrict__ gA, int nA, double* __restrict__ outA,
                                                    const double* __restrict__ gB, int nB, double* __restrict__ outB, int P) {
  __shared__ double red[XW_ADAM_GROUPS][XW_ADAM_PARAMS];
  const double* __restrict__ gslab = blockIdx.y == 0 ? gA : gB;
  const int nslab = blockIdx.y == 0 ? nA : nB;
  double* __restrict__ out = blockIdx.y == 0 ? outA : outB;
  const int tx = threadIdx.x % XW_ADAM_PARAMS, ty = threadIdx.x / XW_ADAM_PARAMS;
  const int i = blockIdx.x * XW_ADAM_PARAMS + tx;
  double a = 0.0;
  if (i < P)
    for (int s = ty; s < nslab; s += XW_ADAM_GROUPS) a += gslab[(long)s * P + i];
  red[ty][tx] = a;
  __syncthreads();
  if (ty != 0 || i >= P) return;
  double g = 0.0;
#pragma unroll 8
  for (int k = 0; k < XW_ADAM_GROUPS; ++k) g += red[k][tx];
  out[i] = g;
}
}
extern "C" int xw_slab_sum2(const double* gA, int nA, double* outA, const double* gB, int nB, double* outB, int P, void* stream) {
  if (!gA || !gB || !outA || !outB || P <= 0 || nA <= 0 || nB <= 0) return XW_E_ARG;
  hipLaunchKernelGGL(k_slab_sum2, dim3((P + XW_ADAM_PARAMS - 1) / XW_ADAM_PARAMS, 2), dim3(XW_ADAM_PARAMS * XW_ADAM_GROUPS), 0,
                     (hipStream_t)stream, gA, nA, outA, gB, nB, outB, P);
  return xw_launch_status();
}

extern "C" int xw_slab_sum(const double* gslab, int nslab, int P, int accumulate, double* out, void* stream) {
  if (!gslab || !out || P <= 0 || nslab <= 0) return XW_E_ARG;
  hipLaunchKernelGGL(k_slab_sum, dim3((P + XW_ADAM_PARAMS - 1) / XW_ADAM_PARAMS), dim3(XW_ADAM_PARAMS * XW_ADAM_GROUPS), 0,
                     (hipStream_t)stream, gslab, nslab, P, accumulate, out);
  return xw_launch_status();
}

extern "C" int xw_abi_version(void) { return 33; }
extern "C" int xw_reduce_work_size(void) { return XW_REDUCE_TICKET + 8; }

extern "C" int xw_supported_dims(char* buf, int buflen) {
  static const char s[] = "ode (H,K)=(20,10),(32,12),(64,16), m=1..10 [MFMA]; any other H<=64, K<=16, m<=32 [generic path: vector ALU, slow]; disc_fwd W=50,64,96,128 any q; disc_bwd W=50 (q=9 unrolled, any q from the record), W=64,96,128 (from the record) [MFMA]; any other W<=128, q<=16 [generic path, from the record]; disc W<=256, q<=32 beyond those [tiled MFMA family, from the record]; d<=126";
  int i = 0;
  for (; s[i] && i < buflen - 1; ++i) buf[i] = s[i];
  if (buflen > 0) buf[i] = 0;
  return i;
}

extern "C" int xw_theta_size(int d, int H, int K) { return u_offsets(d, H, K).total; }
extern "C" int xw_phi_size(int d, int W) { return v_offsets(d, W).total; }

extern "C" int xw_weak_contract_general(const double* A0, int amode, const double* B0, const double* gx, const double* gs,
                                        const double* ghT, const double* gxv, const double* w0, const double* gwx0T,
                                        const double* v0, int d, int N, double* s3x, void* stream) {
  if (!gx || !gs || !ghT || !gxv || !w0 || !gwx0T || !v0 || !s3x || d <= 0 || N <= 0 || amode < 0 || amode > 3 ||
      (amode != 0 && !A0))
    return XW_E_ARG;
  hipLaunchKernelGGL(k_weak_contract, dim3((N + 255) / 256), dim3(256), 0, (hipStream_t)stream, A0, amode, B0, gx, gs, ghT, gxv,
                     w0, gwx0T, v0, d, N, s3x);
  return xw_launch_status();
}
```

xnode_wan_pde_solver_amd/engine.py:

```python
import contextlib
import math
import os

import torch

from . import kernels as KN
from ._lib import XnwanError
from .options import EngineOptions
from .sampling import HIP_HOST_LOCK, _PIN_POOL, Hypercube, _paths


def ctypes_addr(fn):
    import ctypes
    return ctypes.cast(fn, ctypes.c_void_p).value

_KEPT_GRAPHS = []

_NOSTREAM = contextlib.nullcontext()

_SCRATCH_POOL = []


_DEVICE_STREAMS = {}

# ... 94 lines not shown
        self.adjoint = bool(config.get('adjoint', False))
        self.alpha = float(config['alpha'])
        self.pollution = 1.0
        self.verify_structure = opt.verify_structure
        self.packed_load = opt.packed_load
        self.refill_variants = 8
        self.verify_every = 16
        sp = setup.get('shape_param', [-1, 1])
        lo, hi = (sp[0], sp[1]) if isinstance(sp, (list, tuple)) else (-sp, sp)
        self.structure = structure if structure is not None else Structure(funcs, self.d, lo, hi)
        if u_mod.blob is None or v_mod.blob is None:
            raise XnwanError('bind() the networks to the device before building the engine')
        (self.H, self.K), self.m = u_mod.kdims, config['u_layers']
        self.W, self.q = v_mod.kwidth, config['v_layers']
        self.stepper = KN.stepper_family(config['u_hidden_dim'], config['u_hidden_hidden_dim'], self.m, opt.tiled_stepper, self.method)
        self.tiled = self.stepper == 'tiled'
        if self.method == KN.ADAMS and self.adjoint:
            from .nets import ADAMS_ADJOINT_REFUSED
            raise XnwanError(ADAMS_ADJOINT_REFUSED)
        if self.tiled:
            if (self.H, self.K) != (config['u_hidden_dim'], config['u_hidden_hidden_dim']):
                raise XnwanError('the tiled stepper family reads theta at the network\'s own widths; the module was bound at %s'
                                 % ((self.H, self.K),))
            if self.adjoint:
                raise XnwanError('adjoint=True (the continuous adjoint) is not served by the tiled stepper family (u_hidden_dim = %d, '
                                 'u_hidden_hidden_dim = %d, u_layers = %d: it reverses the steps taken; the continuous adjoint exists '
                                 'for the MFMA containers %s, u_layers <= %d)' % (self.H, self.K, self.m, KN.ODE_WIDTHS, KN.ODE_MAX_DEPTH))
            if self.dopri5 and self.dopri5_stepper != 'tiled':
                raise XnwanError("solver 'dopri5' is not served by the tiled stepper family (u_hidden_dim = %d, u_hidden_hidden_dim = %d, "
                                 "u_layers = %d): its field code is the generic path's, up to %s and u_layers %d; the tiled family runs "
                                 "the fixed-grid solvers %s -- unless EngineOptions.dopri5_stepper = 'tiled' (XW_DOPRI5_STEPPER) selects "
                                 "dopri5's implementation on that family" % (self.H, self.K, self.m, KN.GENERIC_ODE_MAX,
                                                                              KN.GENERIC_ODE_MAX_DEPTH, sorted(KN.METHODS)))
        self.testnet = getattr(v_mod, 'family', None) or KN.testnet_family(config['v_hidden_dim'], self.q)
        self.testnet_tiled = self.testnet == 'tiled'
        if self.testnet_tiled and self.W != config['v_hidden_dim']:
            raise XnwanError('the tiled test-network family reads phi at the network\'s own width; the module was bound at %d' % self.W)
        self.generic = (self.stepper == 'generic', not self.testnet_tiled and KN.disc_generic(self.W))
        if any(self.generic):
            import warnings
            which = ' and '.join(n_ for n_, g_ in zip(('u_theta (u_hidden_dim %d, u_hidden_hidden_dim %d, u_layers %d)' % (self.H, self.K, self.m),
                                                       'v_phi (v_hidden_dim %d)' % self.W), self.generic) if g_)
            warnings.warn('%s is outside the MFMA kernel instantiations %s (u_layers <= 10) / %s: running on the generic vector-ALU path, expect a step '
                          'rate lower by two to three orders of magnitude' % (which, KN.ODE_WIDTHS, KN.DISC_WIDTHS), RuntimeWarning, stacklevel=3)
        self.xproj_min_d = 1 << 30 if (self.generic[1] or self.testnet_tiled) else int(opt.xproj_min_d)
        if self.W > 64 and not self.generic[1] and not self.testnet_tiled:
            self.xproj_min_d = 0
        self.xproj_cached = bool(opt.xproj_cached) and self.xproj_min_d < (1 << 30)
        self.xproj_table_min_d = min(self.xproj_min_d, int(opt.xproj_cached_min_d)) if self.xproj_cached else self.xproj_min_d
        if self.generic[0] and self.adjoint:
            raise XnwanError('adjoint=True (the continuous adjoint) exists for the MFMA stepper instantiations %s only; u_hidden_dim = %d, '
                             'u_hidden_hidden_dim = %d run on the generic path, which reverses the steps taken (adjoint=False)'
                             % (KN.ODE_WIDTHS, self.H, self.K))
        self.theta, self.phi = u_mod.blob, v_mod.blob
        self.Pu, self.Pv = self.theta.data.numel(), self.phi.data.numel()
        z = lambda n: torch.zeros(n, dtype=F64, device=device)
        self.adam_u = dict(m=z(self.Pu), v=z(self.Pu), step=torch.zeros(1, dtype=torch.int64, device=device),
                           lag=torch.zeros(1, dtype=torch.int64, device=device))
        self.pairwise_single_slice = opt.pairwise_single_slice
        self.adam_skips_untouched = opt.adam_skips_untouched
        self.eager_checked = 10 ** 12 if opt.always_check else 256
        self.field_range = (self.theta.slots[6][0], self.theta.slots[-2][0])
        self._field_touched = False
        self.adam_v = dict(m=z(self.Pv), v=z(self.Pv), step=torch.zeros(1, dtype=torch.int64, device=device))
        self.grad_u, self.grad_v = z(self.Pu), z(self.Pv)
        self.pack_u = z(2 * self.Pu + 16)
        self.scal = self.pack_u[2 * self.Pu:]
        self.accum_u = self.accum_v = None
        self.use_streams = opt.use_streams
        self.use_graphs = opt.use_graphs
        self.reuse_test_net = opt.reuse_test_net
        self.keep_activations = opt.keep_activations
        cus = torch.cuda.get_device_properties(device).multi_processor_count
        self.v_blocks = int(opt.v_blocks) or (12 * 2 * cus) // 16
        self.v_blocks_disc = int(opt.v_blocks_disc) or (13 * 2 * cus) // 16
        self.narrow = str(opt.narrow)
        if opt.hw_queues > 4:
            import warnings
            warnings.warn('GPU_MAX_HW_QUEUES=%s: the sub-step schedule is tuned for the runtime default of 4 hardware queues and '
                          'measures ~45 %% slower with more' % opt.hw_queues, RuntimeWarning, stacklevel=2)
        self.early_slab_sum = opt.early_slab_sum
        self.compact_tiles = int(opt.compact_tiles)
        self.merged_sweep = bool(opt.merged_sweep)
        self.prio_drop = {'A': int(opt.prio_drop_A) if opt.prio_drop_A is not None else (3 if self.d <= 32 else 2),
                          'X': int(opt.prio_drop_X), 'F': int(opt.prio_drop_F), 'G': int(opt.prio_drop_G)}
        self.use_runner = opt.use_runner
        if self.dopri5:
            self.use_graphs = self.use_streams = self.use_runner = self.keep_activations = False
        if self.tiled:
            self.use_runner = self.keep_activations = False
            self.narrow = '0'
        if self.testnet_tiled:
            self.use_runner = False
        self.narrow_set = str(opt.narrow_set)
        self.narrow_tiles = {'f': 192, 'x': 128, 'p': 64}
        if opt.narrow_tiles:
            self.narrow_tiles = dict(zip('fxp', (int(v_) for v_ in str(opt.narrow_tiles).split(':'))))
        self.narrow_tiles_alone = dict(zip('fxp', (int(v_) for v_ in str(opt.narrow_tiles_alone).split(':'))))
        for k_ in 'fxp':
            self.narrow_tiles_alone[k_] = max(self.narrow_tiles_alone[k_], self.narrow_tiles[k_])
        self.simds = 4 * cus
        self._phi_version = 0
        self.streams, self._cap = _device_streams(device)
        self.capture_exchange = (world is not None and getattr(world, 'capturable', False)
                                 and opt.capture_exchange)
        if self.capture_exchange:
            world.all_reduce(self.scal)

    def _tabulate_a(self, X1):
        d, dev, fa = self.d, self.dev, self.funcs['a']
        N = X1.shape[0]
        A = None
        try:
            ii = torch.arange(d, device=X1.device).view(d, 1, 1, 1)
            jj = torch.arange(d, device=X1.device).view(1, d, 1, 1)
            out = fa(X1.unsqueeze(0).unsqueeze(0), ii, jj)
            if torch.is_tensor(out) and tuple(out.shape) == (d, d, N, 1):
                A = out[..., 0].to(dev).to(F32).to(F64)
                g = torch.Generator().manual_seed(d * 7919 + N)
                for _ in range(3):
                    i, j = (int(k) for k in torch.randint(0, d, (2,), generator=g))
                    if not torch.equal(A[i, j], fa(X1, i, j).to(dev).to(F32).to(F64)[:, 0]):
                        A = None
                        break
        except Exception:
            A = None
        if A is None:
            A = torch.stack([torch.stack([fa(X1, i, j).to(dev).to(F32).to(F64)[:, 0] for j in range(d)], 0) for i in range(d)], 0)
        off = A.clone()
        off.diagonal(dim1=0, dim2=1).zero_()
        if bool(torch.all(A == A[:, :, :1])):
            return A[:, :, 0].contiguous(), 1
        if bool(torch.all(off == 0)):
            return A.diagonal(dim1=0, dim2=1).t().contiguous(), 2
        return A.contiguous(), 3

    def _tabulate_b(self, X1):
        d, dev, fb = self.d, self.dev, self.funcs['b']
        N = X1.shape[0]
        try:
            out = fb(X1.unsqueeze(0), torch.arange(d, device=X1.device).view(d, 1, 1))
            if torch.is_tensor(out) and tuple(out.shape) == (d, N, 1):
                B = out[..., 0].to(dev).to(F32).to(F64)
                if all(torch.equal(B[i], fb(X1, i).to(dev).to(F32).to(F64)[:, 0]) for i in (0, d // 2, d - 1)):
                    return B.contiguous()
        except Exception:
            pass
        return torch.stack([fb(X1, i).to(dev).to(F32).to(F64)[:, 0] for i in range(d)], 0).contiguous()

    def _check_structure(self, X, version):
        st, d = self.structure, self.d
        X1 = X[:, :1, :]
        bad = []
        if st.a_identity:
            for i in range(d):
                j = (i + 1 + version % max(d - 1, 1)) % d
                bad.append(('func_a[%d,%d] == 1' % (i, i), torch.any(self.funcs['a'](X1, i, i) != 1)))
                if d > 1:
                    bad.append(('func_a[%d,%d] == 0' % (i, j), torch.any(self.funcs['a'](X1, i, j) != 0)))
        if st.b_zero:
            for i in range(d):
                bad.append(('func_b[%d] == 0' % i, torch.any(self.funcs['b'](X1, i) != 0)))
        if st.c_kappa is not None:
            key = (tuple(X.shape[:2]), str(X.device))
            if getattr(self, '_probe_u', (None, None))[0] != key:
                g = torch.Generator().manual_seed(1)
# ... 571 lines not shown
                return 0
            except BaseException as e:
                self._exchange_error = e
                return -4
        return EXCHANGE_FN(exchange)

    def _runner_group(self, G):
        from ._lib import XwGroup
        xg = getattr(G, '_xw_group', None)
        if xg is None:
            xg = G._xw_group = XwGroup()
            p = lambda t: 0 if t is None else t.data_ptr()
            xg.N, xg.Nb, xg.L, xg.Lb, xg.d = G.N, G.Nb, G.L, G.Lb, self.d
            xg.same_grid, xg.w_per_point, xg.amode = int(bool(G.same_grid)), int(G.w.dim() == 2), int(G.amode)
            xg.ns_u, xg.ns_b = G.ns_u, G.ns_b
            for k in ('xT', 'xvT', 'xbT', 't', 'tb', 'tpp', 'xvT_pts', 'start', 'start_b', 'h', 'href', 'f', 'g', 'w', 'wt', 'w0', 'ghT',
                      'gwx0T', 'A0', 'B0', 'u', 'Y', 'act', 'act_b', 'v', 'vt', 'gxv', 'gtv', 'gx', 'gs', 'vbar', 's3x', 'vact',
                      'xproj', 'slabA', 'slabB', 'slab_v', 'work_i', 'work_b', 'ub', 'Yb'):
                setattr(xg, k, G.ptr(k))
            nar = lambda jobs, **kw: self._narrow_ok(jobs, **kw)
            ji, jb = self._job(G, 'i'), (self._job(G, 'b') if G.Nb else None)
            joint = G.Nb and G.same_grid
            bits = [nar([ji] + ([jb] if joint else []), alone=False, forward=True),
                    bool(jb) and nar([jb], alone=False, forward=True),
                    nar([ji] + ([jb] if joint else []) + [ji], alone=False),
                    bool(jb) and nar([jb], alone=False),
                    bool(joint) and nar([ji, jb], alone=False),
                    nar([ji], alone=False, params=False),
                    nar([ji], alone=False, forward=True),
                    nar([ji], alone=False, params=False)]
            xg.narrow = sum(1 << i for i, b in enumerate(bits) if b)
        xg.sharded = int(bool(getattr(G, 'sharded', False)))
        xg.xproj_current = (2 if getattr(G, 'xproj_cur', False) else 1) if self._xproj_held(G) else 0
        xg.pair_i, xg.pair_b = int(bool(G.pair_i)), int(bool(G.pair_b))
        xg.Vol, xg.Nglob, xg.Nbglob, xg.s3_scale = float(G.Vol), float(G.Nglob), float(G.Nbglob), float(G.s3_scale)
        xg.init_off, xg.bdry_off, xg.ckappa = float(G.init_off), float(G.bdry_off), float(self.structure.c_kappa)
        xg.href = 0 if G.href is None else G.href.data_ptr()
        xg.c = xg.cp = 0
        return xg

    def _runner_ok(self, G):
        return (self.use_runner and self.structure.c_kappa is not None and G.c is None and not getattr(G, 'persistent', True))

    def _world_of(self, G):
        return self.world if getattr(G, 'sharded', self.world is not None) else None

    def _field_seen(self, G):
        touched = G.L > 1 or (getattr(G, 'has_bdry', G.Nb > 0) and G.Lb > 1)
        self._field_touched = touched or (self.accum_u is not None and self._field_touched)
        return self._field_touched

    def _narrow_ok(self, jobs, alone, forward=False, params=True):
        kind = 'f' if forward else ('p' if params else 'x')
        if self.narrow == '0' or kind not in self.narrow_set:
            return False
        if not forward and (self.adjoint or self.method > 1 or any(j.get('act') is None for j in jobs)):
            return False
        if self.narrow == '2':
            return True
        tiles = sum((j['xT'].shape[1] + 15) // 16 for j in jobs)
        return tiles <= (self.narrow_tiles_alone if alone else self.narrow_tiles)[kind]

    def _job(self, G, which, ubar=None, gslab=None, want_x=False):
        if which == 'i':
            j = dict(xT=G.xT, start=G.start, u=G.u, Y=G.Y, act=G.act, ubar=ubar, gslab=gslab)
            if want_x:
                j.update(gx=G.gx, gs=G.gs)
        else:
            j = dict(xT=G.xbT, start=G.start_b, u=G.ub, Y=G.Yb, act=G.act_b, ubar=ubar, gslab=gslab)
        return j

    def _res_init(self, G):
        return dict(u=G.u, ref=G.href if G.pair_i else G.h, coef=2.0 * self.alpha / G.Nglob, base=self.pollution, first_only=True)

    def _res_bdry(self, G):
        return dict(u=G.ub, ref=G.g, coef=2.0 * self.alpha / (G.Nbglob * G.Lb), base=0.0, first_only=False)

    def _res_weak(self, G):
        return dict(u=G.u, ref=G.v, coef=G.Vol / G.Nglob / G.L * G.s3_scale, base=G.Vol / G.Nglob, weak=dict(w=G.w, c=G.c, cp=G.cp, ckappa=G.ck))

    def _res_merged(self, G):
        return dict(self._res_weak(G), merged=dict(self._res_init(G), scal=self.scal))

    def _contract(self, G, adam_state=None, with_bdry=False):
        fin = None
        if self._world_of(G) is None and adam_state is not None:
            fin = dict(Lb=G.Lb, Nbglob=G.Nbglob, alpha=self.alpha, step=adam_state['step'], init_off=G.init_off, bdry_off=G.bdry_off)
        pair = dict(href=G.href, s3_scale=G.s3_scale) if G.pair_i else None
        bdry = dict(ub=G.ub, g=G.g) if (with_bdry and G.Nb) else None
        if G.A0 is None and G.B0 is None:
            KN.weak_partials(G.u, G.v, G.vt, G.w, G.f, G.h, G.Vol, G.Nglob, self.scal, G.work_i, c=G.c, ckappa=G.ck, wt=G.wt,
                             contract=dict(gx=G.gx, gs=G.gs, ghT=G.ghT, gxv=G.gxv, w0=G.w0, gwx0T=G.gwx0T), finalize=fin, pair=pair,
                             bdry=bdry)
            return
        KN.weak_contract_general(G.A0, G.amode, G.B0, G.gx, G.gs, G.ghT, G.gxv, G.w0, G.gwx0T, G.v[0], G.s3x)
        KN.weak_partials(G.u, G.v, G.vt, G.w, G.f, G.h, G.Vol, G.Nglob, self.scal, G.work_i, s3x=G.s3x, c=G.c, ckappa=G.ck,
                         wt=G.wt, finalize=fin, pair=pair, bdry=bdry)

    def _gen_all(self, G):
        self._gen_front(G)
        self._gen_back(G)

    def _gen_front(self, G):
        th = self.theta.data
        M = (self.method, self.H, self.K, self.m)
        e0 = self._mark()
        fused_x = self.pollution == 1.0 and not self.adjoint
        joint = G.Nb and G.same_grid
        e_x = None
        G.merged = self._merged_ok(G, fused_x, joint)
        if G.merged:
            return self._gen_front_merged(G)
        if self._compact(G, fused_x, joint):
            return self._gen_front_compact(G)
        if not getattr(G, 'skip_v', False):
            self._launch_test_net_here(G)
        with self._side(1, e0):
            fwd = [self._job(G, 'i')] + ([self._job(G, 'b')] if joint else [])
            self._ode_fwd_multi(fwd, G.t, th, *M, zero16=self.scal, narrow=self._narrow_ok(fwd, alone=False, forward=True),
                             prio_drop=self.prio_drop['G'])
            if G.Nb and not joint:
                fwd_b = [self._job(G, 'b')]
                self._ode_fwd_multi(fwd_b, G.tb, th, *M, narrow=self._narrow_ok(fwd_b, alone=False, forward=True))
            self._reaction(G)
            e_f = self._mark()
            e_b = None
            if not fused_x:
                with self._side(2, e_f):
                    sweep_x = [self._job(G, 'i', want_x=True)]
                    self._ode_bwd_multi(sweep_x, G.t, th, *M, want_x=True, want_params=False, adjoint=self.adjoint,
                                     narrow=self._narrow_ok(sweep_x, alone=False, params=False))
                    e_x = self._mark()
            sweeps = [dict(self._job(G, 'i', None, G.slabA[:G.ns_u], want_x=fused_x), res=self._res_init(G))]
            if joint:
                sweeps.append(dict(self._job(G, 'b', None, G.slabA[G.ns_u:]), res=self._res_bdry(G)))
            self._ode_bwd_multi(sweeps, G.t, th, *M, want_x=fused_x, want_params=True, x_cot_ones=fused_x, adjoint=self.adjoint,
                             narrow=self._narrow_ok(sweeps, alone=False), prio_drop=self.prio_drop['A'])
            if G.Nb and not joint:
                sweep_b = [dict(self._job(G, 'b', None, G.slabA[G.ns_u:]), res=self._res_bdry(G))]
                self._ode_bwd_multi(sweep_b, G.tb, th, *M, want_x=False, want_params=True, adjoint=self.adjoint,
                                 narrow=self._narrow_ok(sweep_b, alone=False))
            e_A = self._mark()
            G.sumA_ready = self.early_slab_sum and self._world_of(G) is None and self.accum_u is None and self.use_streams
            e_S = None
            if G.sumA_ready:
                if getattr(G, 'sumA', None) is None:
                    G.sumA = torch.empty(self.Pu, dtype=F64, device=self.dev)
                KN.slab_sum(G.slabA, out=G.sumA)
                e_S = self._mark()
        e_v = self._mark()
        self._join(e_f)
        sweep_B = [dict(self._job(G, 'i', None, G.slabB), res=self._res_weak(G))]
        self._ode_bwd_multi(sweep_B, G.t, th, *M, want_x=False, want_params=True, adjoint=self.adjoint,
                         narrow=self._narrow_ok(sweep_B, alone=True))
        with self._side(3, e_A, e_v, *[e for e in (e_x, e_b) if e is not None]):
            self._contract(G, self.adam_u, with_bdry=True)
            e_C = self._mark()
        self._join(e_C, e_S)

    def _compact(self, G, fused_x, joint):
        tiles = (G.N + 15) // 16 + ((G.Nb + 15) // 16 if G.Nb else 0)
        if not (self.compact_tiles > 0 and self.use_streams and fused_x and joint):
            return False
        return tiles <= self.compact_tiles or bool(getattr(G, 'skip_v', False))

    def _gen_front_compact(self, G):
        th = self.theta.data
        M = (self.method, self.H, self.K, self.m)
        e0 = self._mark()
        if not getattr(G, 'skip_v', False):
            self._launch_test_net_here(G)
        with self._side(1, e0):
            fwd = [self._job(G, 'i'), self._job(G, 'b')]
            lone = bool(getattr(G, 'skip_v', False))
            self._ode_fwd_multi(fwd, G.t, th, *M, zero16=self.scal, narrow=self._narrow_ok(fwd, alone=lone, forward=True),
                             prio_drop=self.prio_drop['G'])
            self._reaction(G)
            e_f = self._mark()
        self._join(e_f)
        sweeps = [dict(self._job(G, 'i', None, G.slabA[:G.ns_u], want_x=True), res=self._res_init(G)),
# ... 116 lines not shown
        from ._lib import check
        self._exchange_error = None
        rc = fn(*args)
        if getattr(self, '_exchange_error', None) is not None:
            err, self._exchange_error = self._exchange_error, None
            raise err
        check(rc, fn.__name__)

    def generator_step(self, G):
        try:
            self._generator_step(G)
        except BaseException:
            G.xproj_key = None
            raise
        finally:
            G.xproj_cur = False

    def _generator_step(self, G):
        sfx = self._v_fresh(G)
        world = self._world_of(G)
        if self._runner_ok(G):
            from ._lib import lib
            skip = self.adam_skips_untouched and not self._field_seen(G)
            G.ck = self.structure.c_kappa
            self._run_runner(lib.xw_substep_gen, self._runner_group(G), self._runner_state(), int(bool(G.skip_v)),
                             int(bool(getattr(G, 'vact_valid', False))), KN._p(self.accum_u), int(skip), KN._stream())
            return
        if world is None:
            self._run(G, 'gen' + sfx, self._gen_all)
            return
        if self.capture_exchange:
            self._run(G, 'gen_dist' + sfx, self._gen_all_dist)
            return
        self._run(G, 'gen_front' + sfx, self._gen_front_packed)
        world.all_reduce(self.pack_u)
        self._run(G, 'gen_back', self._gen_back)

    def _gen_all_dist(self, G):
        self._gen_front_packed(G)
        self.world.all_reduce(self.pack_u)
        self._gen_back(G)

    def _gen_front_packed(self, G):
        P = self.Pu
        if G.N == 0:
            return self._gen_front_empty(G)
        self._gen_front(G)
        KN.slab_sum2(G.slabA, self.pack_u[:P], G.slabB, self.pack_u[P:2 * P])

    def _gen_front_empty(self, G):
        P, th = self.Pu, self.theta.data
        M = (self.method, self.H, self.K, self.m)
        self.pack_u.zero_()
        if not G.Nb:
            return
        fwd_b = [self._job(G, 'b')]
        self._ode_fwd_multi(fwd_b, G.tb, th, *M, narrow=self._narrow_ok(fwd_b, alone=False, forward=True))
        sweep_b = [dict(self._job(G, 'b', None, G.slabA[G.ns_u:]), res=self._res_bdry(G))]
        self._ode_bwd_multi(sweep_b, G.tb, th, *M, want_x=False, want_params=True, adjoint=self.adjoint,
                         narrow=self._narrow_ok(sweep_b, alone=False))
        KN.bdry_partials(G.ub, G.g, self.alpha, G.Nbglob, self.scal, G.work_b)
        KN.slab_sum(G.slabA[G.ns_u:], out=self.pack_u[:P])

    def _disc_front(self, G):
        th = self.theta.data
        M = (self.method, self.H, self.K, self.m)
        if G.N == 0:
            self.scal.zero_()
            return
        e0 = self._mark()
        if not getattr(G, 'skip_v', False):
            self._launch_test_net_here(G, blocks=self.v_blocks_disc)
        with self._side(1, e0):
            fwd = [self._job(G, 'i')]
            lone = bool(getattr(G, 'skip_v', False))
            self._ode_fwd_multi(fwd, G.t, th, *M, zero16=self.scal, act_x_only=True, narrow=self._narrow_ok(fwd, alone=lone, forward=True),
                             prio_drop=self.prio_drop['F'])
            self._reaction(G)
            sweep_x = [self._job(G, 'i', want_x=True)]
            self._ode_bwd_multi(sweep_x, G.t, th, *M, want_x=True, want_params=False, adjoint=self.adjoint,
                             narrow=self._narrow_ok(sweep_x, alone=lone, params=False), prio_drop=self.prio_drop['X'])
            e_x = self._mark()
        self._join(e_x)
        self._contract(G, self.adam_v)

    def _disc_mid(self, G):
        KN.disc_cotangent(G.u, G.v, G.w, G.f, G.h, G.Vol, G.Nglob, self.scal, G.vbar, c=G.c, ckappa=G.ck,
                          pollution=self.pollution, s3_scale=G.s3_scale)
        act = G.vact if getattr(G, 'vact_valid', False) else None
        if G.tpp is None:
            KN.disc_bwd(G.xvT, G.t, self.phi.data, G.vbar, self.W, self.q, gslab=G.slab_v, act=act)
        else:
            KN.disc_bwd(G.xvT_pts, None, self.phi.data, G.vbar.view(1, -1), self.W, self.q, tpp=G.tpp, gslab=G.slab_v, act=act)

    def _disc_mid_packed(self, G):
        if G.N == 0:
            self.grad_v.zero_()
            return
        self._disc_mid(G)
        KN.slab_sum(G.slab_v, out=self.grad_v)

    def _disc_back(self, G):
        lr, st = self.config['v_rate'], self.adam_v
        acc = self.accum_v
        world = self._world_of(G)
        if world is not None:
            KN.losses(self.scal, G.L, G.Lb, G.Vol, G.Nglob, G.Nbglob, self.alpha, step=st['step'])
        if world is None:
            KN.adam(self.phi.data, G.slab_v, st['m'], st['v'], st['step'], lr, gextraA=acc, gsum_out=self.grad_v,
                    bump_step=-1)
        else:
            if acc is not None:
                self.grad_v.add_(acc)
            KN.adam(self.phi.data, None, st['m'], st['v'], st['step'], lr, gextraA=self.grad_v, bump_step=-1)
        if self._xproj_tail(G):
            KN.disc_xproj(G.xvT, self.phi.data, self.W, out=G.xproj)
        if acc is not None:
            acc.copy_(self.grad_v)

    def _reduce_sums(self, G):
        self.world.all_reduce(self.scal[0:9])
        if G.pair_i:
            KN.pair_fold(self.scal, G.Vol, G.Nglob)

    def _disc_all(self, G):
        self._disc_front(G)
        self._disc_mid(G)
        self._disc_back(G)

    def _disc_all_dist(self, G):
        self._disc_front(G)
        self._reduce_sums(G)
        self._disc_mid_packed(G)
        self.world.all_reduce(self.grad_v)
        self._disc_back(G)

    def discriminator_step(self, G):
        try:
            self._discriminator_step(G)
        except BaseException:
            G.xproj_key = None
            raise
        finally:
            G.xproj_cur = False

    def _disc_bookkeeping(self, G):
        sfx = self._v_fresh(G, store=True)
        self._phi_version += 1
        if self._xproj_tail(G):
            G.xproj_key = self._v_key(G)
        return sfx

    def _discriminator_step(self, G):
        sfx = self._disc_bookkeeping(G)
        world = self._world_of(G)
        if self._runner_ok(G):
            from ._lib import lib
            G.ck = self.structure.c_kappa
            self._run_runner(lib.xw_substep_disc, self._runner_group(G), self._runner_state(), int(bool(G.skip_v)),
                             int(bool(getattr(G, 'vact_valid', False))), KN._p(self.accum_v), KN._stream())
            return
        if world is None:
            self._run(G, 'disc' + sfx, self._disc_all)
            return
        if self.capture_exchange:
            self._run(G, 'disc_dist' + sfx, self._disc_all_dist)
            return
        self._run(G, 'disc_front' + sfx, self._disc_front)
        self._reduce_sums(G)
        self._run(G, 'disc_mid' + ('_act' if getattr(G, 'vact_valid', False) else ''), self._disc_mid_packed)
        world.all_reduce(self.grad_v)
        self._run(G, 'disc_back', self._disc_back)

    def _run(self, G, key, fn, scratch=False):
        capturable = (self.use_graphs and self.accum_u is None and self.accum_v is None and getattr(G, 'persistent', True)
                      and not (G.pair_i or G.pair_b))
        g = G.graphs.get(key) if capturable else False
        if g is False:
            if not getattr(G, 'persistent', True) and self.use_streams:
                self.use_streams = False
                self._eager_seen = getattr(self, '_eager_seen', 0) + 1
                KN.TRUSTED = self._eager_seen > self.eager_checked
                try:
                    fn(G)
                finally:
                    self.use_streams = True
                    KN.TRUSTED = False
                return
            fn(G)
            return
        if g is None:
            ran_eager = self.structure.c_kappa is None
            if ran_eager:
                fn(G)
            g = torch.cuda.CUDAGraph()
            torch.cuda.synchronize()
            try:
                with HIP_HOST_LOCK, torch.cuda.graph(g, pool=_scratch_pool(int(scratch) - 1) if scratch else None, stream=self._capture_stream(),
                                                     capture_error_mode='thread_local'):
                    fn(G)
            except Exception as exc:
                if self.options.strict_graphs:
                    raise
                import warnings
                warnings.warn('HIP graph capture of sub-step segment %r failed (%s: %s); this segment now runs as eager kernel launches '
                              '(expect a several times lower step rate)' % (key, type(exc).__name__, exc), RuntimeWarning, stacklevel=2)
                G.graphs[key] = False
                self.eager_segments = getattr(self, 'eager_segments', 0) + 1
                torch.cuda.synchronize()
                if not ran_eager:
                    fn(G)
                return
            G.graphs[key] = g
            _KEPT_GRAPHS.append(g)
            if len(_KEPT_GRAPHS) in (256, 1024, 4096):
                import warnings
                warnings.warn('%d captured HIP graphs are being kept alive (destroying one faults a later launch on this runtime, '
                              'engine._KEPT_GRAPHS): a long-lived process that keeps building solvers should run them with '
                              'XW_GRAPHS=0 or in child processes' % len(_KEPT_GRAPHS), RuntimeWarning, stacklevel=3)
            if ran_eager:
                return
        with HIP_HOST_LOCK:
            g.replay()

    def _capture_stream(self):
        return self._cap

    def loss_u(self):
        return self.scal[4]

    def loss_v(self):
        return self.scal[5]

    def _ode_fwd_multi(self, jobs, t, th, method, H, K, m, zero16=None, **kw):
        if self.tiled and method != KN.DOPRI5:
            return KN.tiled_ode_fwd_multi(jobs, t, th, method, H, K, m, zero16=zero16, **kw)
        if method != KN.DOPRI5:
            return KN.ode_fwd_multi(jobs, t, th, method, H, K, m, zero16=zero16, **kw)
        if zero16 is not None:
            zero16.zero_()
        o = self.options
        for i in range(0, len(jobs), KN.DOPRI5_MAXJOBS):
            part = jobs[i:i + KN.DOPRI5_MAXJOBS]
# ... 55 lines not shown
```

xnode_wan_pde_solver_amd/kernels.py:

```python
import torch

from ._lib import lib, check, XnwanError, XwOdeFwdJob, XwOdeBwdJob, XwDopriJob, XwDopriSweepJob, XwPathsJob, XwPathsDopriJob

METHODS = {'euler': 0, 'midpoint': 1, 'rk4': 2}
DOPRI5 = 3
ADAMS = 4
ADAPTIVE_REFUSED = ('dopri8', 'bosh3', 'fehlberg2', 'adaptive_heun', 'adams', 'implicit_adams',
                    'fixed_adams', 'scipy_solver')
F32, F64 = torch.float32, torch.float64


def _need_gpu():
    if not torch.cuda.is_available():
        raise XnwanError('no GPU visible: the XNODE-WAN kernels only run on an MI355X (gfx950); there is no CPU path')


TRUSTED = False
LONE_NARROW = __import__('os').environ.get('XW_LONE_NARROW', '1') == '1'


def _chk(t, dtype, shape, name):
    if t is None or TRUSTED:
        return
    if not (torch.is_tensor(t) and t.is_cuda):
# ... 605 lines not shown
    check(min(r, 0), 'xw_disc_act_rows')
    return r


def disc_act_view(act, W, q):
    rows = disc_act_rows(W, q)
    return act.reshape(-1)[:act.numel()].view(act.shape[1] // 16, rows, 16)


def disc_act_cols(P):
    return (P + 15) // 16 * 16


def disc_xproj_rows(W):
    return 128 if W > 96 else 96 if W > 64 else 64


def disc_xproj(xT, phi, W, out=None):
    _need_gpu()
    d, N = xT.shape
    _chk(xT, F64, (d, N), 'xT'); _chk(phi, F64, (phi_size(d, W),), 'phi')
    rows = disc_xproj_rows(W)
    out = torch.empty(rows, N, dtype=F64, device=xT.device) if out is None else out
    _chk(out, F64, (rows, N), 'xproj')
    check(lib.xw_disc_xproj(_p(xT), _p(phi), N, d, W, _p(out), _stream()), 'xw_disc_xproj')
    return out


def disc_fwd(xT, t, phi, W, q, tpp=None, want_vt=True, v=None, vt=None, gxv=None, gtv=None, ngrad=0, max_blocks=0, act=None,
             xproj=None, family=None):
    family = _disc_family(W, q, family)
    _need_gpu()
    d, N = xT.shape
    L = 1 if tpp is not None else t.shape[0]
    _chk(xT, F64, (d, N), 'xT'); _chk(phi, F64, (phi_size(d, W),), 'phi')
    _chk(t, F64, None, 't'); _chk(tpp, F64, (N,), 'tpp')
    v = torch.empty(L, N, dtype=F64, device=xT.device) if v is None else v
    if want_vt and vt is None:
        vt = torch.empty(L, N, dtype=F64, device=xT.device)
    _chk(v, F64, (L, N), 'v'); _chk(vt, F64, (L, N), 'vt')
    if gxv is not None:
        _chk(gxv, F64, (d, ngrad), 'gxv'); _chk(gtv, F64, (ngrad,), 'gtv')
    if act is not None:
        _chk(act, F64, (disc_act_rows(W, q, family), disc_act_cols(L * N)), 'act')
    if family == 'tiled':
        if xproj is not None:
            raise XnwanError('the tiled test-network family takes no x-projection table')
        check(lib.xw_disc_tiled_fwd(_p(xT), _p(t), _p(tpp), _p(phi), N, L, d, W, q, _p(v), _p(vt if want_vt else None), _p(gxv),
                                    _p(gtv), int(ngrad), int(max_blocks), _p(act), None, _stream()), 'xw_disc_tiled_fwd')
        return v, (vt if want_vt else None)
    if xproj is not None:
        _chk(xproj, F64, (disc_xproj_rows(W), N), 'xproj')
    check(lib.xw_disc_fwd_xproj(_p(xT), _p(t), _p(tpp), _p(phi), N, L, d, W, q, _p(v), _p(vt if want_vt else None), _p(gxv),
                                _p(gtv), int(ngrad), int(max_blocks), _p(act), _p(xproj), _stream()), 'xw_disc_fwd')
    return v, (vt if want_vt else None)


def disc_gradx(xT, t, phi, W, q, tpp=None, vbar=None, gxv=None, gtv=None, family=None):
    family = _disc_family(W, q, family)
    _need_gpu()
    d, N = xT.shape
    _chk(xT, F64, (d, N), 'xT'); _chk(phi, F64, (phi_size(d, W),), 'phi'); _chk(t, F64, None, 't'); _chk(tpp, F64, (N,), 'tpp')
    gxv = torch.empty(d, N, dtype=F64, device=xT.device) if gxv is None else gxv
    gtv = torch.empty(N, dtype=F64, device=xT.device) if gtv is None else gtv
    _chk(gxv, F64, (d, N), 'gxv'); _chk(gtv, F64, (N,), 'gtv')
    if vbar is not None:
        vbar = vbar.reshape(-1)
        _chk(vbar, F64, (N,), 'vbar')
    if family == 'tiled' or not disc_recompute(W, q):
        t0 = t[:1] if tpp is None else None
        disc_fwd(xT, t0, phi, W, q, tpp=tpp, want_vt=False, gxv=gxv, gtv=gtv, ngrad=N, family=family)
        if vbar is not None:
            gxv.mul_(vbar)
            gtv.mul_(vbar)
        return gxv, gtv
    check(lib.xw_disc_gradx(_p(xT), _p(t), _p(tpp), _p(phi), _p(vbar), N, d, W, q, _p(gxv), _p(gtv), _stream()), 'xw_disc_gradx')
    return gxv, gtv


def disc_bwd_slabs(N, L):
    return lib.xw_disc_bwd_slabs(N, L)


def disc_bwd(xT, t, phi, vbar, W, q, tpp=None, gslab=None, act=None, family=None):
    family = _disc_family(W, q, family)
    _need_gpu()
    d, N = xT.shape
    L = 1 if tpp is not None else t.shape[0]
    P = phi_size(d, W)
    _chk(xT, F64, (d, N), 'xT'); _chk(phi, F64, (P,), 'phi'); _chk(vbar, F64, (L, N), 'vbar')
    _chk(t, F64, None, 't'); _chk(tpp, F64, (N,), 'tpp')
    ns = disc_bwd_slabs(N, L)
    gslab = torch.empty(ns, P, dtype=F64, device=xT.device) if gslab is None else gslab
    _chk(gslab, F64, (ns, P), 'gslab')
    if act is None and (family == 'tiled' or not disc_recompute(W, q)):
        act = torch.empty(disc_act_rows(W, q, family), disc_act_cols(L * N), dtype=F64, device=xT.device)
        disc_fwd(xT, t, phi, W, q, tpp=tpp, want_vt=False, act=act, family=family)
    if act is not None:
        _chk(act, F64, (disc_act_rows(W, q, family), disc_act_cols(L * N)), 'act')
    if family == 'tiled':
        check(lib.xw_disc_tiled_bwd(_p(xT), _p(t), _p(tpp), _p(phi), _p(vbar), N, L, d, W, q, _p(act), _p(gslab), _stream()),
              'xw_disc_tiled_bwd')
        return gslab
    check(lib.xw_disc_bwd(_p(xT), _p(t), _p(tpp), _p(phi), _p(vbar), N, L, d, W, q, _p(act), _p(gslab), _stream()),
          'xw_disc_bwd')
    return gslab


def reduce_work_size():
    return lib.xw_reduce_work_size()


def weak_partials(u, v, vt, w, f, h, Vol, Nglob, scal, work, s3x=None, contract=None, c=None, ckappa=0.0, wt=None,
                  finalize=None, pair=None, bdry=None):
    _need_gpu()
    L, N = u.shape
    for name, a in (('u', u), ('v', v), ('vt', vt), ('f', f)):
        _chk(a, F64, (L, N), name)
    per_point = 1 if w.dim() == 2 else 0
    _chk(w, F64, (L, N) if per_point else (N,), 'w'); _chk(wt, F64, (L, N), 'wt'); _chk(c, F64, (L, N), 'c')
    _chk(s3x, F64, (N,), 's3x'); _chk(h, F64, (N,), 'h'); _chk(scal, F64, (16,), 'scal')
    _chk(work, F64, (reduce_work_size(),), 'work')
    fz = finalize or {}
    _chk(fz.get('step'), torch.int64, (1,), 'step')
    bd, Pb = bdry or {}, 0
    if bdry is not None:
        Pb = bdry['ub'].numel()
        _chk(bdry['ub'], F64, tuple(bdry['ub'].shape), 'ub'); _chk(bdry['g'], F64, tuple(bdry['ub'].shape), 'g')
    pr = pair or {}
    _chk(pr.get('href'), F64, (N,), 'href')
    if pair is not None and L != 1:
        raise XnwanError('the pairwise form only exists for single-slice groups (L == 1)')
    k, d = {}, 0
    if s3x is None:
        k = contract
        d = k['gx'].shape[0]
        for name in ('gx', 'ghT', 'gxv', 'gwx0T'):
            _chk(k[name], F64, (d, N), name)
        _chk(k['gs'], F64, (N,), 'gs'); _chk(k['w0'], F64, (N,), 'w0')
    check(lib.xw_weak_partials(_p(u), _p(v), _p(vt), _p(w), per_point, _p(wt), _p(s3x), _p(k.get('gx')), _p(k.get('gs')),
                               _p(k.get('ghT')), _p(k.get('gxv')), _p(k.get('w0')), _p(k.get('gwx0T')), d, _p(c),
                               float(ckappa), _p(f), _p(h), _p(pr.get('href')), 0 if pair is None else 1,
                               float(pr.get('s3_scale', 1.0)), N, L, float(Vol), float(Nglob), _p(work), _p(scal),
                               0 if finalize is None else 1, max(int(fz.get('Lb', 1)), 1), float(fz.get('Nbglob', 1.0)),
                               float(fz.get('alpha', 0.0)), float(fz.get('init_off', 0.0)), float(fz.get('bdry_off', 0.0)),
                               _p(fz.get('step')), _p(bd.get('ub')), _p(bd.get('g')), Pb, _stream()),
          'xw_weak_partials')


def pair_fold(scal, Vol, Nglob):
    _need_gpu()
    _chk(scal, F64, (16,), 'scal')
    check(lib.xw_pair_fold(_p(scal), float(Vol), float(Nglob), _stream()), 'xw_pair_fold')


def cube_weight(x, top, bot, w, gwT, w0=None, xT=None):
    _need_gpu()
    N, d = x.shape
    _chk(x, torch.float32, (N, d), 'x')
    _chk(w, F64, (N,), 'w')
    _chk(gwT, F64, (d, N), 'gwT')
    if w0 is not None:
        _chk(w0, F64, (N,), 'w0')
    if xT is not None:
        _chk(xT, F64, (d, N), 'xT')
    check(lib.xw_cube_weight(_p(x), N, d, float(top), float(bot), _p(w), _p(w0), _p(gwT), _p(xT), _stream()), 'xw_cube_weight')


GATHER_ROWS = 1024


def gather_fields(table, count, total):
    _need_gpu()
    if table.dtype != torch.int64 or table.dim() != 2 or table.shape[1] != 9 or not table.is_contiguous() or table.shape[0] < count:
        raise XnwanError('gather table: need a contiguous int64 [>= count, 9] device tensor')
    check(lib.xw_gather_fields(_p(table), int(count), int(total), _stream()), 'xw_gather_fields')


def weak_contract_general(A0, amode, B0, gx, gs, ghT, gxv, w0, gwx0T, v0, s3x):
    _need_gpu()
    d, N = gx.shape
    for name, a in (('gx', gx), ('ghT', ghT), ('gxv', gxv), ('gwx0T', gwx0T)):
        _chk(a, F64, (d, N), name)
    for name, a in (('gs', gs), ('w0', w0), ('v0', v0), ('s3x', s3x)):
        _chk(a, F64, (N,), name)
    _chk(B0, F64, (d, N), 'B0')
    amode = int(amode)
    if amode not in (0, 1, 2, 3) or (amode == 0) != (A0 is None):
        raise XnwanError('weak_contract_general: amode %r does not match A0' % (amode,))
    if amode:
        _chk(A0, F64, {1: (d, d), 2: (d, N), 3: (d, d, N)}[amode], 'A0')
    check(lib.xw_weak_contract_general(_p(A0), amode, _p(B0), _p(gx), _p(gs), _p(ghT), _p(gxv), _p(w0), _p(gwx0T), _p(v0), d, N,
                                       _p(s3x), _stream()), 'xw_weak_contract_general')
    return s3x


def bdry_partials(ub, g, alpha, Nbglob, scal, work, ubar_b=None):
    _need_gpu()
    L, Nb = ub.shape
    _chk(ub, F64, (L, Nb), 'ub'); _chk(g, F64, (L, Nb), 'g'); _chk(ubar_b, F64, (L, Nb), 'ubar_b'); _chk(scal, F64, (16,), 'scal')
    _chk(work, F64, (reduce_work_size(),), 'work')
    check(lib.xw_bdry_partials(_p(ub), _p(g), Nb, L, float(alpha), float(Nbglob), _p(ubar_b), _p(work), _p(scal), _stream()),
          'xw_bdry_partials')


def gen_cotangents(u, v, w, h, Vol, Nglob, alpha, ubarA, ubarB, c=None, cp=None, ckappa=0.0, pollution=1.0, scal=None):
    _need_gpu()
    if ubarA is None and ubarB is None:
        raise XnwanError('gen_cotangents: nothing to compute')
    L, N = u.shape
    per_point = 1 if w.dim() == 2 else 0
    _chk(u, F64, (L, N), 'u'); _chk(v, F64, (L, N), 'v'); _chk(w, F64, (L, N) if per_point else (N,), 'w')
    _chk(c, F64, (L, N), 'c'); _chk(cp, F64, (L, N), 'cp'); _chk(h, F64, (N,), 'h')
    _chk(ubarA, F64, (L, N), 'ubarA'); _chk(ubarB, F64, (L, N), 'ubarB'); _chk(scal, F64, (16,), 'scal')
    check(lib.xw_gen_cotangents(_p(u), _p(v), _p(w), per_point, _p(c), _p(cp), float(ckappa), _p(h), N, L, float(Vol),
                                float(Nglob), float(alpha), float(pollution), _p(scal), _p(ubarA), _p(ubarB), _stream()),
          'xw_gen_cotangents')


def disc_cotangent(u, v, w, f, h, Vol, Nglob, scal, vbar, c=None, ckappa=0.0, pollution=1.0, s3_scale=1.0):
    _need_gpu()
    L, N = u.shape
    per_point = 1 if w.dim() == 2 else 0
    _chk(u, F64, (L, N), 'u'); _chk(v, F64, (L, N), 'v'); _chk(w, F64, (L, N) if per_point else (N,), 'w')
    _chk(c, F64, (L, N), 'c'); _chk(f, F64, (L, N), 'f'); _chk(h, F64, (N,), 'h'); _chk(vbar, F64, (L, N), 'vbar')
    _chk(scal, F64, (16,), 'scal')
    check(lib.xw_disc_cotangent(_p(u), _p(v), _p(w), per_point, _p(c), float(ckappa), _p(f), _p(h), N, L, float(Vol),
                                float(Nglob), float(pollution), float(s3_scale), _p(scal), _p(vbar), _stream()), 'xw_disc_cotangent')


def losses(scal, L, Lb, Vol, Nglob, Nbglob, alpha, step=None, init_off=0.0, bdry_off=0.0):
    _need_gpu()
    _chk(scal, F64, (16,), 'scal'); _chk(step, torch.int64, (1,), 'step')
    check(lib.xw_losses(_p(scal), L, max(int(Lb), 1), float(Vol), float(Nglob), float(Nbglob), float(alpha), float(init_off),
                        float(bdry_off), _p(step), _stream()), 'xw_losses')


def adam(param, gslabA, m, v, step, lr, beta1=0.9, beta2=0.999, eps=1e-8, gextraA=None, gslabB=None, gextraB=None,
         scal=None, gsum_out=None, bump_step=True, lag=None, lag_range=(0, 0), skip=False):
    _need_gpu()
    P = param.shape[0]
    _chk(param, F64, (P,), 'param'); _chk(m, F64, (P,), 'm'); _chk(v, F64, (P,), 'v'); _chk(step, torch.int64, (1,), 'step')
    nA = nB = 0
    if gslabA is not None:
        nA = gslabA.shape[0]
        _chk(gslabA, F64, (nA, P), 'gslabA')
    if gslabB is not None:
        nB = gslabB.shape[0]
        _chk(gslabB, F64, (nB, P), 'gslabB')
    _chk(gextraA, F64, (P,), 'gextraA'); _chk(gextraB, F64, (P,), 'gextraB'); _chk(gsum_out, F64, (P,), 'gsum_out')
    _chk(scal, F64, (16,), 'scal'); _chk(lag, torch.int64, (1,), 'lag')
    lo, hi = (int(lag_range[0]), int(lag_range[1])) if lag is not None else (0, 0)
    check(lib.xw_adam(_p(param), _p(gslabA), nA, _p(gextraA), _p(gslabB), nB, _p(gextraB), _p(scal), _p(m), _p(v), _p(step),
                      (1 if bump_step is True else 0 if bump_step is False else int(bump_step)), P,
                      float(lr), float(beta1), float(beta2), float(eps), _p(gsum_out), lo, hi, 1 if skip else 0, _p(lag),
                      _stream()), 'xw_adam')


def slab_sum2(gA, outA, gB, outB):
    _need_gpu()
    (nA, P), (nB, P2) = gA.shape, gB.shape
    _chk(gA, F64, (nA, P), 'gA'); _chk(gB, F64, (nB, P), 'gB'); _chk(outA, F64, (P,), 'outA'); _chk(outB, F64, (P,), 'outB')
    check(lib.xw_slab_sum2(_p(gA), nA, _p(outA), _p(gB), nB, _p(outB), P, _stream()), 'xw_slab_sum2')


def slab_sum(gslab, out=None, accumulate=False):
    _need_gpu()
    ns, P = gslab.shape
    _chk(gslab, F64, (ns, P), 'gslab')
    out = torch.empty(P, dtype=F64, device=gslab.device) if out is None else out
    _chk(out, F64, (P,), 'out')
    check(lib.xw_slab_sum(_p(gslab), ns, P, 1 if accumulate else 0, _p(out), _stream()), 'xw_slab_sum')
    return out
```

xnode_wan_pde_solver_amd/options.py:

```python
import dataclasses
import os
from typing import Optional


def _flag(name, default):
    v = os.environ.get(name)
    if v is None:
        return default
    return v != '0' if default else v == '1'


def _int(name, default):
    v = os.environ.get(name)
    return default if v in (None, '') else int(v)


@dataclasses.dataclass
class EngineOptions:
    use_streams: bool = True
    use_graphs: bool = True
    strict_graphs: bool = False
    reuse_test_net: bool = False
    keep_activations: bool = True
    v_blocks: int = 0
    v_blocks_disc: int = 0
    narrow: str = '1'
    narrow_set: str = 'fx'
    narrow_tiles: Optional[str] = None
    narrow_tiles_alone: str = '256:256:64'
    early_slab_sum: bool = True
    merged_sweep: bool = True
    compact_tiles: int = 320
    prio_drop_A: Optional[int] = None
    prio_drop_X: int = 0
    prio_drop_F: int = 0
    prio_drop_G: int = 0
    use_runner: bool = True
    capture_exchange: bool = True
    xproj_min_d: int = 45
    xproj_cached: bool = True
    xproj_cached_min_d: int = 20
    tiled_stepper: str = 'beyond'
    eval_chunk_paths: int = 65536
    hw_queues: int = 4
    verify_structure: bool = True
    packed_load: bool = True
    pairwise_single_slice: bool = True
    adam_skips_untouched: bool = True
    always_check: bool = False
    poison: bool = False
    capture_refill: bool = True
    defer_list_readback: bool = True
    sampler_process: bool = True
    show_plan: bool = False
    dopri5_chunk: int = 8
    dopri5_max_steps: int = 10000
    dopri5_stepper: str = 'vector'
    replicate_below: int = 16
    native_allreduce: bool = True

    @classmethod
    def from_env(cls):
        o = cls()
        o.use_streams = _flag('XW_STREAMS', o.use_streams)
        o.use_graphs = _flag('XW_GRAPHS', o.use_graphs)
        o.strict_graphs = _flag('XW_STRICT_GRAPHS', o.strict_graphs)
        o.reuse_test_net = _flag('XW_REUSE_V', o.reuse_test_net)
        o.keep_activations = _flag('XW_KEEP_ACT', o.keep_activations)
        o.v_blocks = _int('XW_V_BLOCKS', o.v_blocks)
        o.v_blocks_disc = _int('XW_V_BLOCKS_DISC', o.v_blocks_disc)
        o.narrow = os.environ.get('XW_NARROW', o.narrow)
        o.narrow_set = os.environ.get('XW_NARROW_SET', o.narrow_set)
        o.narrow_tiles = os.environ.get('XW_NARROW_TILES') or None
        o.narrow_tiles_alone = os.environ.get('XW_NARROW_TILES_ALONE') or o.narrow_tiles_alone
        o.early_slab_sum = _flag('XW_EARLY_SLAB_SUM', o.early_slab_sum)
        o.merged_sweep = _flag('XW_MERGED_SWEEP', o.merged_sweep)
        o.compact_tiles = _int('XW_COMPACT_TILES', o.compact_tiles)
        o.prio_drop_A = _int('XW_PRIO_DROP_A', None)
        o.prio_drop_X = _int('XW_PRIO_DROP_X', o.prio_drop_X)
        o.prio_drop_F = _int('XW_PRIO_DROP_F', o.prio_drop_F)
        o.prio_drop_G = _int('XW_PRIO_DROP_G', o.prio_drop_G)
        o.use_runner = _flag('XW_RUNNER', o.use_runner)
        o.capture_exchange = _flag('XW_CAPTURE_EXCHANGE', o.capture_exchange)
        o.xproj_min_d = _int('XW_XPROJ_MIN_D', o.xproj_min_d)
        o.xproj_cached = _flag('XW_XPROJ_CACHED', o.xproj_cached)
        o.xproj_cached_min_d = _int('XW_XPROJ_CACHED_MIN_D', o.xproj_cached_min_d)
        o.tiled_stepper = os.environ.get('XW_TILED_STEPPER') or o.tiled_stepper
        o.eval_chunk_paths = _int('XW_EVAL_CHUNK_PATHS', o.eval_chunk_paths)
        try:
            o.hw_queues = _int('GPU_MAX_HW_QUEUES', o.hw_queues)
        except ValueError:
            pass
        o.verify_structure = _flag('XW_VERIFY_STRUCTURE', o.verify_structure)
        o.packed_load = _flag('XW_PACKED_LOAD', o.packed_load)
        o.pairwise_single_slice = not _flag('XW_ELEMENTWISE_SINGLE_SLICE', False)
        o.adam_skips_untouched = not _flag('XW_ADAM_NO_SKIP', False)
        o.always_check = _flag('XW_ALWAYS_CHECK', o.always_check)
        o.poison = _flag('XW_POISON', o.poison)
        o.capture_refill = _flag('XW_CAPTURE_REFILL', o.capture_refill)
        o.defer_list_readback = _flag('XW_DEFER_LIST', o.defer_list_readback)
        o.sampler_process = _flag('XW_SAMPLER_PROCESS', o.sampler_process)
        o.show_plan = _flag('XW_SHOW_PLAN', o.show_plan)
        o.dopri5_chunk = _int('XW_DOPRI5_CHUNK', o.dopri5_chunk)
        o.dopri5_max_steps = _int('XW_DOPRI5_MAX_STEPS', o.dopri5_max_steps)
        o.dopri5_stepper = os.environ.get('XW_DOPRI5_STEPPER') or o.dopri5_stepper
        o.replicate_below = _int('XW_REPLICATE_BELOW', o.replicate_below)
        o.native_allreduce = _flag('XW_NATIVE_ALLREDUCE', o.native_allreduce)
        return o

    def non_default(self):
        base = EngineOptions()
        return {f.name: getattr(self, f.name) for f in dataclasses.fields(self) if getattr(self, f.name) != getattr(base, f.name)}
```

Baseline: 2209.

## Fuse discriminator cotangent into weak-partials basis and record backward kernel

The weak-partials contraction now writes a per-point dI basis, and the recorded discriminator backward kernel combines it with v, w and the scalar reductions to form vbar on the fly. This removes the separate xw_disc_cotangent pass and its vbar read and write. In exchange the backward kernel does extra global loads of v, w and scal per point and carries pointers staged through LDS. The path is on by default through a new option and falls back when no activation record exists or the width is unsupported.

```diff
diff --git a/include/xnwan_cot.h b/include/xnwan_cot.h
--- /dev/null
+++ b/include/xnwan_cot.h
@@ -0,0 +1,27 @@
+#ifndef XNWAN_COT_H
+#define XNWAN_COT_H
+#include "xnwan.h"
+#ifdef __cplusplus
+extern "C" {
+#endif
+
+int xw_weak_partials_basis(const double* u, const double* v, const double* vt, const double* w, int w_per_point,
+                           const double* wt, const double* s3x, const double* gx, const double* gs, const double* ghT,
+                           const double* gxv, const double* w0, const double* gwx0T, int d, const double* c, double ckappa,
+                           const double* f, const double* h, const double* href, int pairwise, double s3_scale, int N, int L,
+                           double Vol, double Nglob, double* work, double* scal, int finalize, int Lb, double Nbglob, double alpha,
+                           double init_off, double bdry_off, long long* step, const double* ub, const double* gb, long Pb,
+                           double cot_s3_scale, double* dI_basis, void* stream);
+int xw_disc_cot_combine(const double* dI_basis, const double* v, const double* w, int w_per_point, int N, int L,
+                        double pollution, const double* scal_in, double* vbar, void* stream);
+int xw_disc_bwd_basis_ok(int W, int have_record);
+int xw_disc_bwd_basis(const double* xT, const double* t, const double* tpp, const double* phi, const double* dI_basis,
+                      const double* v, const double* w, int w_per_point, int Nw, double pollution, const double* scal,
+                      int N, int L, int d, int W, int q, const double* act, double* gslab, void* stream);
+int xw_substep_disc_form(const XwGroup* g, const XwSolverState* s, int skip_v, int use_record, double* accum, int basis,
+                         void* stream);
+
+#ifdef __cplusplus
+}
+#endif
+#endif
diff --git a/xnode_wan_pde_solver_amd/_lib.py b/xnode_wan_pde_solver_amd/_lib.py
--- a/xnode_wan_pde_solver_amd/_lib.py
+++ b/xnode_wan_pde_solver_amd/_lib.py
@@ -158,6 +158,15 @@
                             c_int, c_f64p, c_vp],
 }
 
+COT_SIGNATURES = {
+    'xw_weak_partials_basis': SIGNATURES['xw_weak_partials'][:-1] + [c_dbl, c_f64p, c_vp],
+    'xw_disc_cot_combine': [c_f64p, c_f64p, c_f64p, c_int, c_int, c_int, c_dbl, c_f64p, c_f64p, c_vp],
+    'xw_disc_bwd_basis_ok': [c_int, c_int],
+    'xw_disc_bwd_basis': [c_f32p, c_f32p, c_f32p, c_f64p, c_f64p, c_f64p, c_f64p, c_int, c_int, c_dbl, c_f64p, c_int, c_int, c_int,
+                          c_int, c_int, c_f64p, c_f64p, c_vp],
+    'xw_substep_disc_form': [ctypes.POINTER(XwGroup), ctypes.POINTER(XwSolverState), c_int, c_int, c_f64p, c_int, c_vp],
+}
+
 ERRORS = {-1: 'XW_E_DIMS: network widths/depths not among the compiled kernel instantiations',
           -2: 'XW_E_ARG: null pointer, non-positive size or bad enum',
           -3: 'XW_E_WORKSPACE: workspace too small',
@@ -175,7 +184,7 @@
             'or `make -C xnode_wan_pde_solver_amd/csrc`.  There is no CPU fallback.' % LIB_PATH)
     import torch
     lib = ctypes.CDLL(LIB_PATH)
-    for name, argtypes in list(SIGNATURES.items()) + list(EVAL_SIGNATURES.items()):
+    for name, argtypes in list(SIGNATURES.items()) + list(EVAL_SIGNATURES.items()) + list(COT_SIGNATURES.items()):
         fn = getattr(lib, name)
         fn.argtypes = argtypes
         fn.restype = ctypes.c_int
diff --git a/xnode_wan_pde_solver_amd/csrc/xw_cot.h b/xnode_wan_pde_solver_amd/csrc/xw_cot.h
--- /dev/null
+++ b/xnode_wan_pde_solver_amd/csrc/xw_cot.h
@@ -0,0 +1,27 @@
+#pragma once
+
+struct XwCotCoef {
+  double cN, K;
+};
+__device__ __forceinline__ XwCotCoef xw_cot_coef(double Vol, double Nglob, int L, double s3_scale) {
+#pragma clang fp contract(off)
+  XwCotCoef k;
+  k.cN = Vol / Nglob;
+  k.K = __dmul_rn(Vol / Nglob / (double)L, s3_scale);
+  return k;
+}
+
+__device__ __forceinline__ double xw_cot_dI(const XwCotCoef k, double ul, double cl, double fp, double wl, bool last, bool first,
+                                            double hn) {
+#pragma clang fp contract(off)
+  double dI = __dmul_rn(__dmul_rn(k.K, fma(ul, cl, fp)), wl);
+  if (last) dI = fma(k.cN, ul, dI);
+  if (first) dI = fma(-k.cN, hn, dI);
+  return dI;
+}
+
+__device__ __forceinline__ double xw_cot_vbar(double pollution, double wl, double dI, double vl, double I, double S) {
+#pragma clang fp contract(off)
+  const double cI = __ddiv_rn(2.0, I);
+  return __dadd_rn(fma(pollution, wl, -__dmul_rn(cI, dI)), __ddiv_rn(__dadd_rn(vl, vl), S));
+}
diff --git a/xnode_wan_pde_solver_amd/csrc/xw_disc_bwd.hip b/xnode_wan_pde_solver_amd/csrc/xw_disc_bwd.hip
--- a/xnode_wan_pde_solver_amd/csrc/xw_disc_bwd.hip
+++ b/xnode_wan_pde_solver_amd/csrc/xw_disc_bwd.hip
@@ -1,4 +1,5 @@
 #include "xw_disc_core.h"
+#include "xnwan_cot.h"
 #include <cstdlib>
 
 namespace {
@@ -287,6 +288,13 @@
   return {d + 2 <= 48 ? 1 : d + 2 <= 96 ? 2 : 3, tsum_on && !point_mode && (N % 64) == 0};
 }
 
+int launch_from_record(const double* xT, const double* t, const double* tpp, const double* phi, const double* vbar, int N, int L, int d,
+                       int W, int q, const double* act, double* gslab, const XwRecCot& cot, void* stream) {
+  static const bool tsum_on = [] { const char* e = getenv("XW_DISC_REC_TSUM"); return !(e && e[0] == '0'); }();
+  const RecKey k = rec_select(N, d, tpp != nullptr, tsum_on);
+  return xw_disc_rec_launch(W, k.ng, k.tsum, bwd_blocks((long)N * L), xT, t, tpp, phi, vbar, N, L, d, gslab, act, q, cot, stream);
+}
+
 }
 
 extern "C" int xw_disc_bwd_slabs(int N, int L) { return bwd_blocks((long)N * L); }
@@ -299,13 +307,25 @@
   if (!disc_width_ok(W)) return xwg_disc_bwd(xT, t, tpp, phi, vbar, N, L, d, W, q, act, gslab, bwd_blocks((long)N * L), stream);
   if (q < 0 || d + 2 > 128 || ((q != 9 || W != 50) && act == nullptr)) return XW_E_DIMS;
   if ((long)N * L * 4 >= (1L << 31)) return XW_E_ARG;
-  if (act != nullptr) {
-    static const bool tsum_on = [] { const char* e = getenv("XW_DISC_REC_TSUM"); return !(e && e[0] == '0'); }();
-    const RecKey k = rec_select(N, d, tpp != nullptr, tsum_on);
-    return xw_disc_rec_launch(W, k.ng, k.tsum, bwd_blocks((long)N * L), xT, t, tpp, phi, vbar, N, L, d, gslab, act, q, stream);
-  }
+  if (act != nullptr)
+    return launch_from_record(xT, t, tpp, phi, vbar, N, L, d, W, q, act, gslab, XwRecCot{nullptr, nullptr, nullptr, 0.0, 0}, stream);
   launch_recompute(false, xT, t, tpp, phi, vbar, N, L, d, gslab, nullptr, nullptr, stream);
   return xw_launch_status();
+}
+
+extern "C" int xw_disc_bwd_basis_ok(int W, int have_record) { return disc_width_ok(W) && have_record ? 1 : 0; }
+
+extern "C" int xw_disc_bwd_basis(const double* xT, const double* t, const double* tpp, const double* phi, const double* dI_basis,
+                                 const double* v, const double* w, int w_per_point, int Nw, double pollution, const double* scal,
+                                 int N, int L, int d, int W, int q, const double* act, double* gslab, void* stream) {
+  if (!xT || !phi || !gslab || !dI_basis || !v || !w || !scal || N <= 0 || L <= 0 || d <= 0) return XW_E_ARG;
+  if (!tpp && !t) return XW_E_ARG;
+  if (tpp && L != 1) return XW_E_ARG;
+  if (!w_per_point && (Nw <= 0 || (tpp ? N % Nw != 0 : Nw != N))) return XW_E_ARG;
+  if (!disc_width_ok(W) || act == nullptr || q < 0 || d + 2 > 128) return XW_E_DIMS;
+  if ((long)N * L * 4 >= (1L << 31)) return XW_E_ARG;
+  return launch_from_record(xT, t, tpp, phi, dI_basis, N, L, d, W, q, act, gslab,
+                            XwRecCot{v, w, scal, pollution, w_per_point ? 0 : Nw}, stream);
 }
 
 extern "C" int xw_disc_gradx(const double* xT, const double* t, const double* tpp, const double* phi, const double* vbar,
diff --git a/xnode_wan_pde_solver_amd/csrc/xw_disc_core.h b/xnode_wan_pde_solver_amd/csrc/xw_disc_core.h
--- a/xnode_wan_pde_solver_amd/csrc/xw_disc_core.h
+++ b/xnode_wan_pde_solver_amd/csrc/xw_disc_core.h
@@ -66,6 +66,14 @@
 
 }
 
+struct XwRecCot {
+  const double* v;
+  const double* w;
+  const double* scal;
+  double pollution;
+  int wN;
+};
+
 XWG_HIDDEN int xw_disc_rec_launch(int W, int ng, bool tsum, int blocks, const double* xT, const double* t, const double* tpp,
                                   const double* phi, const double* vbar, int N, int L, int d, double* gslab, const double* act,
-                                  int q, void* stream);
+                                  int q, const XwRecCot& cot, void* stream);
diff --git a/xnode_wan_pde_solver_amd/csrc/xw_disc_rec.hip b/xnode_wan_pde_solver_amd/csrc/xw_disc_rec.hip
--- a/xnode_wan_pde_solver_amd/csrc/xw_disc_rec.hip
+++ b/xnode_wan_pde_solver_amd/csrc/xw_disc_rec.hip
@@ -1,4 +1,5 @@
 #include "xw_disc_core.h"
+#include "xw_cot.h"
 
 namespace {
 
@@ -22,7 +23,8 @@
   static constexpr int oR = oD + 4 * wset;
   static constexpr int oO = oR + 4 * wset;
   static constexpr int NO = 4 * D::MT;
-  static constexpr int total = oO + (NO + 1) * 16;
+  static constexpr int oC = oO + (NO + 1) * 16;
+  static constexpr int total = oC + 8;
   static_assert(total * 8 <= (VT ? 80 : 160) * 1024, "two blocks per CU (short tail) / one");
   __device__ static constexpr int toff(int mt) { return mt * XW_TTILE; }
 };
@@ -37,7 +39,8 @@
 __global__ void __launch_bounds__(256, RecLds<W>::VT ? 2 : 1) k_disc_rec(const double* __restrict__ xT, const double* __restrict__ tf,
                                                      const double* __restrict__ tpp, const double* __restrict__ ph,
                                                      const double* __restrict__ vbar, int N, int L, int d,
-                                                     double* __restrict__ gslab, const double* __restrict__ act, int qrt) {
+                                                     double* __restrict__ gslab, const double* __restrict__ act, int qrt,
+                                                     const XwRecCot cot) {
   typedef VDim<W> D;
   typedef RecLds<W> S;
   __shared__ double lds[S::total];
@@ -72,6 +75,14 @@
     }
   if (threadIdx.x < 16 * D::MT) sVo[threadIdx.x] = (int)threadIdx.x < W ? ph[o.Vo + threadIdx.x] : 0.0;
   for (int idx = threadIdx.x; idx < (S::NO + 1) * 16; idx += blockDim.x) sO[idx] = 0.0;
+  double* sC = lds + S::oC;
+  if (threadIdx.x == 0) {
+    sC[0] = __longlong_as_double((long long)cot.v);
+    sC[1] = __longlong_as_double((long long)cot.w);
+    sC[2] = __longlong_as_double((long long)cot.scal);
+    sC[3] = cot.pollution;
+    sC[4] = __longlong_as_double((long long)cot.wN);
+  }
   __syncthreads();
 
   d4 accH[TW * TW], accB[D::MT];
@@ -126,7 +137,15 @@
     d4 a[D::MT], rnext[D::MT];
     load_layer(nq, a);
     if (nq > 0) load_layer(nq - 1, rnext);
-    const double vb = pt.valid ? (vbar != nullptr ? xw_ld_g(vbar + pt.p) : 1.0) : 0.0;
+    double vb = pt.valid ? (vbar != nullptr ? xw_ld_g(vbar + pt.p) : 1.0) : 0.0;
+    const double* cv = (const double*)__double_as_longlong(sC[0]);
+    if (cv != nullptr && pt.valid) {
+      const double* cw = (const double*)__double_as_longlong(sC[1]);
+      const double* cs = (const double*)__double_as_longlong(sC[2]);
+      const int wN = (int)__double_as_longlong(sC[4]);
+      const int wi = wN == 0 ? pt.p : (tpp != nullptr ? (int)((unsigned)pt.p % (unsigned)wN) : pt.n);
+      vb = xw_cot_vbar(sC[3], xw_ld_g(cw + wi), vb, xw_ld_g(cv + pt.p), xw_ld_g(cs), xw_ld_g(cs + 1));
+    }
     d4 dl[D::MT];
 #pragma unroll
     for (int mt = 0; mt < D::MT; ++mt)
@@ -467,7 +486,7 @@
 }
 
 typedef void (*RecKernel)(const double*, const double*, const double*, const double*, const double*, int, int, int, double*,
-                          const double*, int);
+                          const double*, int, const XwRecCot);
 struct RecRow {
   int W;
   RecKernel k[3][2];
@@ -483,12 +502,12 @@
 
 int xw_disc_rec_launch(int W, int ng, bool tsum, int blocks, const double* xT, const double* t, const double* tpp,
                        const double* phi, const double* vbar, int N, int L, int d, double* gslab, const double* act, int q,
-                       void* stream) {
+                       const XwRecCot& cot, void* stream) {
   if (ng < 1 || ng > 3) return XW_E_DIMS;
   for (const RecRow& row : rec_table)
     if (row.W == W) {
       hipLaunchKernelGGL(row.k[ng - 1][tsum ? 1 : 0], dim3(blocks), dim3(256), 0, (hipStream_t)stream, xT, t, tpp, phi, vbar, N, L,
-                         d, gslab, act, q);
+                         d, gslab, act, q, cot);
       return xw_launch_status();
     }
   return XW_E_DIMS;
diff --git a/xnode_wan_pde_solver_amd/csrc/xw_substep.hip b/xnode_wan_pde_solver_amd/csrc/xw_substep.hip
--- a/xnode_wan_pde_solver_amd/csrc/xw_substep.hip
+++ b/xnode_wan_pde_solver_amd/csrc/xw_substep.hip
@@ -1,6 +1,7 @@
 #include <hip/hip_runtime.h>
 #include <string.h>
 #include "xnwan.h"
+#include "xnwan_cot.h"
 
 namespace {
 struct Side {
@@ -43,7 +44,8 @@
   return xw_disc_fwd_xproj(g->xvT, g->t, nullptr, s->phi, g->N, g->L, g->d, s->W, s->q, g->v, g->vt, g->gxv, g->gtv, g->N, blocks, record,
                            g->xproj, stream);
 }
-int contract(const XwGroup* g, const XwSolverState* s, long long* step, bool with_bdry, bool finalize, void* stream) {
+int contract(const XwGroup* g, const XwSolverState* s, long long* step, bool with_bdry, bool finalize, void* stream,
+             double* dI_basis = nullptr) {
   const double* s3x = nullptr;
   if (g->A0 != nullptr || g->B0 != nullptr) {
     XW_TRY(xw_weak_contract_general(g->A0, g->amode, g->B0, g->gx, g->gs, g->ghT, g->gxv, g->w0, g->gwx0T, g->v, g->d, g->N, g->s3x,
@@ -51,12 +53,13 @@
     s3x = g->s3x;
   }
   const bool fused = s3x == nullptr;
-  return xw_weak_partials(g->u, g->v, g->vt, g->w, g->w_per_point, g->wt, s3x, fused ? g->gx : nullptr, fused ? g->gs : nullptr,
+  return xw_weak_partials_basis(g->u, g->v, g->vt, g->w, g->w_per_point, g->wt, s3x, fused ? g->gx : nullptr, fused ? g->gs : nullptr,
                           fused ? g->ghT : nullptr, fused ? g->gxv : nullptr, fused ? g->w0 : nullptr, fused ? g->gwx0T : nullptr,
                           fused ? g->d : 0, g->c, g->ckappa, g->f, g->h, g->pair_i ? g->href : nullptr, g->pair_i ? 1 : 0,
                           g->pair_i ? g->s3_scale : 1.0, g->N, g->L, g->Vol, g->Nglob, g->work_i, s->scal, finalize ? 1 : 0,
                           g->Lb > 0 ? g->Lb : 1, g->Nbglob, s->alpha, g->init_off, g->bdry_off, finalize ? step : nullptr, with_bdry && g->Nb > 0 ? g->ub : nullptr,
-                          with_bdry && g->Nb > 0 ? g->g : nullptr, with_bdry && g->Nb > 0 ? (long)g->Nb * g->Lb : 0, stream);
+                          with_bdry && g->Nb > 0 ? g->g : nullptr, with_bdry && g->Nb > 0 ? (long)g->Nb * g->Lb : 0, g->s3_scale, dI_basis,
+                          stream);
 }
 inline bool sharded(const XwGroup* g, const XwSolverState* s) { return g->sharded != 0 && s->exchange != nullptr; }
 #define XW_ZERO(ptr, count) XW_HIP(hipMemsetAsync((ptr), 0, sizeof(double) * (size_t)(count), (hipStream_t)stream))
@@ -206,7 +209,13 @@
 }
 
 extern "C" int xw_substep_disc(const XwGroup* g, const XwSolverState* s, int skip_v, int use_record, double* accum, void* stream) {
+  return xw_substep_disc_form(g, s, skip_v, use_record, accum, 0, stream);
+}
+
+extern "C" int xw_substep_disc_form(const XwGroup* g, const XwSolverState* s, int skip_v, int use_record, double* accum, int basis,
+                                    void* stream) {
   if (!g || !s || g->N < 0 || g->L <= 0) return XW_E_ARG;
+  const bool cot_basis = basis != 0 && xw_disc_bwd_basis_ok(s->W, use_record) != 0;
   const bool shard = sharded(g, s);
   if (g->N == 0 && !shard) return XW_E_ARG;
   const bool have_i = g->N > 0;
@@ -231,7 +240,7 @@
     XW_HIP(hipEventRecord(sd->done, sd->s));
     stream = main_stream;
     XW_HIP(hipStreamWaitEvent((hipStream_t)main_stream, sd->done, 0));
-    XW_TRY(contract(g, s, s->step_v, false, !shard, stream));
+    XW_TRY(contract(g, s, s->step_v, false, !shard, stream, cot_basis ? g->vbar : nullptr));
   } else {
     XW_ZERO(s->scal, 16);
   }
@@ -240,7 +249,15 @@
     if (g->pair_i) XW_TRY(xw_pair_fold(s->scal, g->Vol, g->Nglob, stream));
   }
   const int nsv = have_i ? xw_disc_bwd_slabs(g->N, g->L) : 0;
-  if (have_i) {
+  if (have_i && cot_basis) {
+    if (g->tpp != nullptr) {
+      XW_TRY(xw_disc_bwd_basis(g->xvT_pts, nullptr, g->tpp, s->phi, g->vbar, g->v, g->w, g->w_per_point, g->N, s->pollution, s->scal,
+                               g->N * g->L, 1, g->d, s->W, s->q, record, g->slab_v, stream));
+    } else {
+      XW_TRY(xw_disc_bwd_basis(g->xvT, g->t, nullptr, s->phi, g->vbar, g->v, g->w, g->w_per_point, g->N, s->pollution, s->scal, g->N,
+                               g->L, g->d, s->W, s->q, record, g->slab_v, stream));
+    }
+  } else if (have_i) {
     XW_TRY(xw_disc_cotangent(g->u, g->v, g->w, g->w_per_point, g->c, g->ckappa, g->f, g->h, g->N, g->L, g->Vol, g->Nglob, s->pollution,
                              g->s3_scale, s->scal, g->vbar, stream));
     if (g->tpp != nullptr) {
diff --git a/xnode_wan_pde_solver_amd/csrc/xw_weak.hip b/xnode_wan_pde_solver_amd/csrc/xw_weak.hip
--- a/xnode_wan_pde_solver_amd/csrc/xw_weak.hip
+++ b/xnode_wan_pde_solver_amd/csrc/xw_weak.hip
@@ -1,5 +1,7 @@
 #include "xw_common.h"
+#include "xw_cot.h"
 #include "xnwan.h"
+#include "xnwan_cot.h"
 
 namespace {
 
@@ -85,10 +87,12 @@
                                                        double* __restrict__ scal, int finalize, int Lb, double Nbglob,
                                                        double alpha, double init_off, double bdry_off,
                                                        long long* __restrict__ step, const double* __restrict__ ub,
-                                                       const double* __restrict__ gb, long Pb) {
+                                                       const double* __restrict__ gb, long Pb, double cot_s3_scale,
+                                                       double* __restrict__ dI_basis) {
   double acc[6] = {0.0, 0.0, 0.0, 0.0, 0.0, 0.0};
   const double cN = Vol / Nglob, cNL = Vol / Nglob / (double)L;
   const long P = (long)N * L;
+  const XwCotCoef cot = xw_cot_coef(Vol, Nglob, L, cot_s3_scale);
   for (long p = (long)blockIdx.x * blockDim.x + threadIdx.x; p < P; p += (long)gridDim.x * blockDim.x) {
     const int l = (int)(p / N), n = (int)(p - (long)l * N);
     const double ul = u[p], vl = v[p];
@@ -98,6 +102,7 @@
     if (wt != nullptr) phit += vl * wt[p];
     const double cl = c != nullptr ? c[p] : ckappa * ul;
     double s3 = cl * ul * phi + f[p] * phi;
+    if (dI_basis != nullptr) dI_basis[p] = xw_cot_dI(cot, ul, cl, f[p], wl, l == L - 1, l == 0, l == 0 ? h[n] : 0.0);
     double I = 0.0;
     if (l == 0) {
       const double hn = h[n];
@@ -236,19 +241,26 @@
                                                   int L, double Vol, double Nglob, double pollution, double s3_scale,
                                                   const double* __restrict__ scal_in, double* __restrict__ vbar) {
   const double I = scal_in[0], S = scal_in[1];
-  const double cI = 2.0 / I;
-  const double cN = Vol / Nglob, cNL = Vol / Nglob / (double)L;
+  const XwCotCoef cot = xw_cot_coef(Vol, Nglob, L, s3_scale);
   const long P = (long)N * L;
   for (long p = (long)blockIdx.x * blockDim.x + threadIdx.x; p < P; p += (long)gridDim.x * blockDim.x) {
     const int l = (int)(p / N), n = (int)(p - (long)l * N);
     const double ul = u[p], vl = v[p];
     const double wl = w_per_point ? w[p] : w[n];
     const double cl = c != nullptr ? c[p] : ckappa * ul;
-    double dI = cNL * s3_scale * (cl * ul + f[p]) * wl;
-    if (l == L - 1) dI += cN * ul;
-    if (l == 0) dI -= cN * h[n];
-    vbar[p] = pollution * wl - cI * dI + 2.0 * vl / S;
-  }
+    const double dI = xw_cot_dI(cot, ul, cl, f[p], wl, l == L - 1, l == 0, l == 0 ? h[n] : 0.0);
+    vbar[p] = xw_cot_vbar(pollution, wl, dI, vl, I, S);
+  }
+}
+
+__global__ void __launch_bounds__(256) k_disc_cot_combine(const double* __restrict__ dI_basis, const double* __restrict__ v,
+                                                          const double* __restrict__ w, int w_per_point, int N, int L,
+                                                          double pollution, const double* __restrict__ scal_in,
+                                                          double* __restrict__ vbar) {
+  const double I = scal_in[0], S = scal_in[1];
+  const long P = (long)N * L;
+  for (long p = (long)blockIdx.x * blockDim.x + threadIdx.x; p < P; p += (long)gridDim.x * blockDim.x)
+    vbar[p] = xw_cot_vbar(pollution, w_per_point ? w[p] : w[p % N], dI_basis[p], v[p], I, S);
 }
 
 #define XW_ADAM_PARAMS 16
@@ -358,6 +370,24 @@
 }
 }
 
+extern "C" int xw_weak_partials_basis(const double* u, const double* v, const double* vt, const double* w, int w_per_point,
+                                      const double* wt, const double* s3x, const double* gx, const double* gs, const double* ghT,
+                                      const double* gxv, const double* w0, const double* gwx0T, int d, const double* c,
+                                      double ckappa, const double* f, const double* h, const double* href, int pairwise,
+                                      double s3_scale, int N, int L, double Vol, double Nglob, double* work, double* scal,
+                                      int finalize, int Lb, double Nbglob, double alpha, double init_off, double bdry_off,
+                                      long long* step, const double* ub, const double* gb, long Pb, double cot_s3_scale,
+                                      double* dI_basis, void* stream) {
+  if (!u || !v || !vt || !w || !f || !h || !work || !scal || N <= 0 || L <= 0 || (finalize && Lb <= 0)) return XW_E_ARG;
+  if ((ub == nullptr) != (gb == nullptr) || (ub != nullptr && Pb <= 0)) return XW_E_ARG;
+  if (!s3x && (!gx || !gs || !ghT || !gxv || !w0 || !gwx0T || d <= 0)) return XW_E_ARG;
+  if (pairwise && L != 1) return XW_E_ARG;
+  hipLaunchKernelGGL(k_weak_partials, dim3(blocks_for((long)N * L, reduce_threads(), reduce_cap((long)N * L))), dim3(reduce_threads()), 0, (hipStream_t)stream, u, v, vt, w,
+                     w_per_point, wt, s3x, gx, gs, ghT, gxv, w0, gwx0T, d, c, ckappa, f, h, href, pairwise, s3_scale, N, L, Vol,
+                     Nglob, work, scal, finalize, Lb, Nbglob, alpha, init_off, bdry_off, step, ub, gb, Pb, cot_s3_scale, dI_basis);
+  return xw_launch_status();
+}
+
 extern "C" int xw_weak_partials(const double* u, const double* v, const double* vt, const double* w, int w_per_point,
                                 const double* wt, const double* s3x, const double* gx, const double* gs, const double* ghT,
                                 const double* gxv, const double* w0, const double* gwx0T, int d, const double* c,
@@ -365,14 +395,9 @@
                                 double s3_scale, int N, int L, double Vol, double Nglob, double* work, double* scal,
                                 int finalize, int Lb, double Nbglob, double alpha, double init_off, double bdry_off,
                                 long long* step, const double* ub, const double* gb, long Pb, void* stream) {
-  if (!u || !v || !vt || !w || !f || !h || !work || !scal || N <= 0 || L <= 0 || (finalize && Lb <= 0)) return XW_E_ARG;
-  if ((ub == nullptr) != (gb == nullptr) || (ub != nullptr && Pb <= 0)) return XW_E_ARG;
-  if (!s3x && (!gx || !gs || !ghT || !gxv || !w0 || !gwx0T || d <= 0)) return XW_E_ARG;
-  if (pairwise && L != 1) return XW_E_ARG;
-  hipLaunchKernelGGL(k_weak_partials, dim3(blocks_for((long)N * L, reduce_threads(), reduce_cap((long)N * L))), dim3(reduce_threads()), 0, (hipStream_t)stream, u, v, vt, w,
-                     w_per_point, wt, s3x, gx, gs, ghT, gxv, w0, gwx0T, d, c, ckappa, f, h, href, pairwise, s3_scale, N, L, Vol,
-                     Nglob, work, scal, finalize, Lb, Nbglob, alpha, init_off, bdry_off, step, ub, gb, Pb);
-  return xw_launch_status();
+  return xw_weak_partials_basis(u, v, vt, w, w_per_point, wt, s3x, gx, gs, ghT, gxv, w0, gwx0T, d, c, ckappa, f, h, href, pairwise,
+                                s3_scale, N, L, Vol, Nglob, work, scal, finalize, Lb, Nbglob, alpha, init_off, bdry_off, step, ub, gb,
+                                Pb, 1.0, nullptr, stream);
 }
 
 extern "C" int xw_bdry_partials(const double* ub, const double* g, int Nb, int L, double alpha, double Nbglob,
@@ -450,6 +475,14 @@
   if (!u || !v || !w || !f || !h || !scal_in || !vbar || N <= 0 || L <= 0) return XW_E_ARG;
   hipLaunchKernelGGL(k_disc_cot, dim3(blocks_for((long)N * L, 256, 2048)), dim3(256), 0, (hipStream_t)stream, u, v, w,
                      w_per_point, c, ckappa, f, h, N, L, Vol, Nglob, pollution, s3_scale, scal_in, vbar);
+  return xw_launch_status();
+}
+
+extern "C" int xw_disc_cot_combine(const double* dI_basis, const double* v, const double* w, int w_per_point, int N, int L,
+                                   double pollution, const double* scal_in, double* vbar, void* stream) {
+  if (!dI_basis || !v || !w || !scal_in || !vbar || N <= 0 || L <= 0) return XW_E_ARG;
+  hipLaunchKernelGGL(k_disc_cot_combine, dim3(blocks_for((long)N * L, 256, 2048)), dim3(256), 0, (hipStream_t)stream, dI_basis, v, w,
+                     w_per_point, N, L, pollution, scal_in, vbar);
   return xw_launch_status();
 }
 
diff --git a/xnode_wan_pde_solver_amd/engine.py b/xnode_wan_pde_solver_amd/engine.py
--- a/xnode_wan_pde_solver_amd/engine.py
+++ b/xnode_wan_pde_solver_amd/engine.py
@@ -200,6 +200,7 @@
         self.early_slab_sum = opt.early_slab_sum
         self.compact_tiles = int(opt.compact_tiles)
         self.merged_sweep = bool(opt.merged_sweep)
+        self.disc_cot_basis = bool(opt.disc_cot_basis)
         self.prio_drop = {'A': int(opt.prio_drop_A) if opt.prio_drop_A is not None else (3 if self.d <= 32 else 2),
                           'X': int(opt.prio_drop_X), 'F': int(opt.prio_drop_F), 'G': int(opt.prio_drop_G)}
         self.use_runner = opt.use_runner
@@ -937,7 +938,8 @@
     def _res_merged(self, G):
         return dict(self._res_weak(G), merged=dict(self._res_init(G), scal=self.scal))
 
-    def _contract(self, G, adam_state=None, with_bdry=False):
+    def _contract(self, G, adam_state=None, with_bdry=False, dI_basis=None):
+        basis = dict(dI_basis=dI_basis, cot_s3_scale=G.s3_scale) if dI_basis is not None else {}
         fin = None
         if self._world_of(G) is None and adam_state is not None:
             fin = dict(Lb=G.Lb, Nbglob=G.Nbglob, alpha=self.alpha, step=adam_state['step'], init_off=G.init_off, bdry_off=G.bdry_off)
@@ -946,11 +948,11 @@
         if G.A0 is None and G.B0 is None:
             KN.weak_partials(G.u, G.v, G.vt, G.w, G.f, G.h, G.Vol, G.Nglob, self.scal, G.work_i, c=G.c, ckappa=G.ck, wt=G.wt,
                              contract=dict(gx=G.gx, gs=G.gs, ghT=G.ghT, gxv=G.gxv, w0=G.w0, gwx0T=G.gwx0T), finalize=fin, pair=pair,
-                             bdry=bdry)
+                             bdry=bdry, **basis)
             return
         KN.weak_contract_general(G.A0, G.amode, G.B0, G.gx, G.gs, G.ghT, G.gxv, G.w0, G.gwx0T, G.v[0], G.s3x)
         KN.weak_partials(G.u, G.v, G.vt, G.w, G.f, G.h, G.Vol, G.Nglob, self.scal, G.work_i, s3x=G.s3x, c=G.c, ckappa=G.ck,
-                         wt=G.wt, finalize=fin, pair=pair, bdry=bdry)
+                         wt=G.wt, finalize=fin, pair=pair, bdry=bdry, **basis)
 
     def _gen_all(self, G):
         self._gen_front(G)
@@ -1233,12 +1235,24 @@
                              narrow=self._narrow_ok(sweep_x, alone=lone, params=False), prio_drop=self.prio_drop['X'])
             e_x = self._mark()
         self._join(e_x)
-        self._contract(G, self.adam_v)
+        self._contract(G, self.adam_v, dI_basis=G.vbar if self._disc_cot_form(G) else None)
+
+    def _disc_cot_form(self, G):
+        return bool(self.disc_cot_basis and not self.testnet_tiled
+                    and KN.disc_bwd_basis_ok(self.W, self.q, getattr(G, 'vact_valid', False) and G.vact is not None))
 
     def _disc_mid(self, G):
+        act = G.vact if getattr(G, 'vact_valid', False) else None
+        if self._disc_cot_form(G):
+            basis = dict(v=G.v, w=G.w, scal=self.scal, pollution=self.pollution)
+            if G.tpp is None:
+                KN.disc_bwd(G.xvT, G.t, self.phi.data, G.vbar, self.W, self.q, gslab=G.slab_v, act=act, basis=basis)
+            else:
+                KN.disc_bwd(G.xvT_pts, None, self.phi.data, G.vbar.view(1, -1), self.W, self.q, tpp=G.tpp, gslab=G.slab_v, act=act,
+                            basis=basis)
+            return
         KN.disc_cotangent(G.u, G.v, G.w, G.f, G.h, G.Vol, G.Nglob, self.scal, G.vbar, c=G.c, ckappa=G.ck,
                           pollution=self.pollution, s3_scale=G.s3_scale)
-        act = G.vact if getattr(G, 'vact_valid', False) else None
         if G.tpp is None:
             KN.disc_bwd(G.xvT, G.t, self.phi.data, G.vbar, self.W, self.q, gslab=G.slab_v, act=act)
         else:
@@ -1308,8 +1322,8 @@
         if self._runner_ok(G):
             from ._lib import lib
             G.ck = self.structure.c_kappa
-            self._run_runner(lib.xw_substep_disc, self._runner_group(G), self._runner_state(), int(bool(G.skip_v)),
-                             int(bool(getattr(G, 'vact_valid', False))), KN._p(self.accum_v), KN._stream())
+            self._run_runner(lib.xw_substep_disc_form, self._runner_group(G), self._runner_state(), int(bool(G.skip_v)),
+                             int(bool(getattr(G, 'vact_valid', False))), KN._p(self.accum_v), int(self.disc_cot_basis), KN._stream())
             return
         if world is None:
             self._run(G, 'disc' + sfx, self._disc_all)
diff --git a/xnode_wan_pde_solver_amd/kernels.py b/xnode_wan_pde_solver_amd/kernels.py
--- a/xnode_wan_pde_solver_amd/kernels.py
+++ b/xnode_wan_pde_solver_amd/kernels.py
@@ -711,14 +711,26 @@
     return lib.xw_disc_bwd_slabs(N, L)
 
 
-def disc_bwd(xT, t, phi, vbar, W, q, tpp=None, gslab=None, act=None, family=None):
+def disc_bwd(xT, t, phi, vbar, W, q, tpp=None, gslab=None, act=None, family=None, basis=None):
     family = _disc_family(W, q, family)
     _need_gpu()
     d, N = xT.shape
     L = 1 if tpp is not None else t.shape[0]
     P = phi_size(d, W)
-    _chk(xT, F64, (d, N), 'xT'); _chk(phi, F64, (P,), 'phi'); _chk(vbar, F64, (L, N), 'vbar')
+    _chk(xT, F64, (d, N), 'xT'); _chk(phi, F64, (P,), 'phi')
     _chk(t, F64, None, 't'); _chk(tpp, F64, (N,), 'tpp')
+    if basis is None:
+        _chk(vbar, F64, (L, N), 'vbar')
+    else:
+        bv, bw = basis['v'], basis['w']
+        Lw, Nw = bv.shape
+        per_point = 1 if bw.dim() == 2 else 0
+        if Lw * Nw != L * N or vbar is None or vbar.numel() != L * N:
+            raise XnwanError('disc_bwd(basis=...): v, the basis and the launch must cover the same %d points' % (L * N))
+        if act is None or not disc_bwd_basis_ok(W, q, True, family):
+            raise XnwanError('disc_bwd(basis=...): the basis form only exists from the record, at the MFMA widths %s' % (DISC_WIDTHS,))
+        _chk(vbar, F64, None, 'dI_basis'); _chk(bv, F64, (Lw, Nw), 'v'); _chk(bw, F64, (Lw, Nw) if per_point else (Nw,), 'w')
+        _chk(basis['scal'], F64, (16,), 'scal')
     ns = disc_bwd_slabs(N, L)
     gslab = torch.empty(ns, P, dtype=F64, device=xT.device) if gslab is None else gslab
     _chk(gslab, F64, (ns, P), 'gslab')
@@ -727,6 +739,11 @@
         disc_fwd(xT, t, phi, W, q, tpp=tpp, want_vt=False, act=act, family=family)
     if act is not None:
         _chk(act, F64, (disc_act_rows(W, q, family), disc_act_cols(L * N)), 'act')
+    if basis is not None:
+        check(lib.xw_disc_bwd_basis(_p(xT), _p(t), _p(tpp), _p(phi), _p(vbar), _p(bv), _p(bw), per_point, Nw,
+                                    float(basis.get('pollution', 1.0)), _p(basis['scal']), N, L, d, W, q, _p(act), _p(gslab), _stream()),
+              'xw_disc_bwd_basis')
+        return gslab
     if family == 'tiled':
         check(lib.xw_disc_tiled_bwd(_p(xT), _p(t), _p(tpp), _p(phi), _p(vbar), N, L, d, W, q, _p(act), _p(gslab), _stream()),
               'xw_disc_tiled_bwd')
@@ -741,9 +758,10 @@
 
 
 def weak_partials(u, v, vt, w, f, h, Vol, Nglob, scal, work, s3x=None, contract=None, c=None, ckappa=0.0, wt=None,
-                  finalize=None, pair=None, bdry=None):
+                  finalize=None, pair=None, bdry=None, dI_basis=None, cot_s3_scale=1.0):
     _need_gpu()
     L, N = u.shape
+    _chk(dI_basis, F64, (L, N), 'dI_basis')
     for name, a in (('u', u), ('v', v), ('vt', vt), ('f', f)):
         _chk(a, F64, (L, N), name)
     per_point = 1 if w.dim() == 2 else 0
@@ -767,14 +785,17 @@
         for name in ('gx', 'ghT', 'gxv', 'gwx0T'):
             _chk(k[name], F64, (d, N), name)
         _chk(k['gs'], F64, (N,), 'gs'); _chk(k['w0'], F64, (N,), 'w0')
-    check(lib.xw_weak_partials(_p(u), _p(v), _p(vt), _p(w), per_point, _p(wt), _p(s3x), _p(k.get('gx')), _p(k.get('gs')),
-                               _p(k.get('ghT')), _p(k.get('gxv')), _p(k.get('w0')), _p(k.get('gwx0T')), d, _p(c),
-                               float(ckappa), _p(f), _p(h), _p(pr.get('href')), 0 if pair is None else 1,
-                               float(pr.get('s3_scale', 1.0)), N, L, float(Vol), float(Nglob), _p(work), _p(scal),
-                               0 if finalize is None else 1, max(int(fz.get('Lb', 1)), 1), float(fz.get('Nbglob', 1.0)),
-                               float(fz.get('alpha', 0.0)), float(fz.get('init_off', 0.0)), float(fz.get('bdry_off', 0.0)),
-                               _p(fz.get('step')), _p(bd.get('ub')), _p(bd.get('g')), Pb, _stream()),
-          'xw_weak_partials')
+    args = (_p(u), _p(v), _p(vt), _p(w), per_point, _p(wt), _p(s3x), _p(k.get('gx')), _p(k.get('gs')),
+            _p(k.get('ghT')), _p(k.get('gxv')), _p(k.get('w0')), _p(k.get('gwx0T')), d, _p(c),
+            float(ckappa), _p(f), _p(h), _p(pr.get('href')), 0 if pair is None else 1,
+            float(pr.get('s3_scale', 1.0)), N, L, float(Vol), float(Nglob), _p(work), _p(scal),
+            0 if finalize is None else 1, max(int(fz.get('Lb', 1)), 1), float(fz.get('Nbglob', 1.0)),
+            float(fz.get('alpha', 0.0)), float(fz.get('init_off', 0.0)), float(fz.get('bdry_off', 0.0)),
+            _p(fz.get('step')), _p(bd.get('ub')), _p(bd.get('g')), Pb)
+    if dI_basis is None:
+        check(lib.xw_weak_partials(*args, _stream()), 'xw_weak_partials')
+    else:
+        check(lib.xw_weak_partials_basis(*args, float(cot_s3_scale), _p(dI_basis), _stream()), 'xw_weak_partials_basis')
 
 
 def pair_fold(scal, Vol, Nglob):
@@ -856,6 +877,20 @@
     _chk(scal, F64, (16,), 'scal')
     check(lib.xw_disc_cotangent(_p(u), _p(v), _p(w), per_point, _p(c), float(ckappa), _p(f), _p(h), N, L, float(Vol),
                                 float(Nglob), float(pollution), float(s3_scale), _p(scal), _p(vbar), _stream()), 'xw_disc_cotangent')
+
+
+def disc_cot_combine(dI_basis, v, w, scal, vbar, pollution=1.0):
+    _need_gpu()
+    L, N = v.shape
+    per_point = 1 if w.dim() == 2 else 0
+    _chk(dI_basis, F64, (L, N), 'dI_basis'); _chk(v, F64, (L, N), 'v'); _chk(w, F64, (L, N) if per_point else (N,), 'w')
+    _chk(vbar, F64, (L, N), 'vbar'); _chk(scal, F64, (16,), 'scal')
+    check(lib.xw_disc_cot_combine(_p(dI_basis), _p(v), _p(w), per_point, N, L, float(pollution), _p(scal), _p(vbar), _stream()),
+          'xw_disc_cot_combine')
+
+
+def disc_bwd_basis_ok(W, q, have_record, family=None):
+    return bool(have_record) and _disc_family(W, q, family) != 'tiled' and bool(lib.xw_disc_bwd_basis_ok(int(W), 1))
 
 
 def losses(scal, L, Lb, Vol, Nglob, Nbglob, alpha, step=None, init_off=0.0, bdry_off=0.0):
diff --git a/xnode_wan_pde_solver_amd/options.py b/xnode_wan_pde_solver_amd/options.py
--- a/xnode_wan_pde_solver_amd/options.py
+++ b/xnode_wan_pde_solver_amd/options.py
@@ -29,6 +29,7 @@
     narrow_tiles: Optional[str] = None
     narrow_tiles_alone: str = '256:256:64'
     early_slab_sum: bool = True
+    disc_cot_basis: bool = True
     merged_sweep: bool = True
     compact_tiles: int = 320
     prio_drop_A: Optional[int] = None
@@ -75,6 +76,7 @@
         o.narrow_tiles_alone = os.environ.get('XW_NARROW_TILES_ALONE') or o.narrow_tiles_alone
         o.early_slab_sum = _flag('XW_EARLY_SLAB_SUM', o.early_slab_sum)
         o.merged_sweep = _flag('XW_MERGED_SWEEP', o.merged_sweep)
+        o.disc_cot_basis = _flag('XW_DISC_COT_BASIS', o.disc_cot_basis)
         o.compact_tiles = _int('XW_COMPACT_TILES', o.compact_tiles)
         o.prio_drop_A = _int('XW_PRIO_DROP_A', None)
         o.prio_drop_X = _int('XW_PRIO_DROP_X', o.prio_drop_X)
```

After: 2214 (median of 3 runs). Within noise of the previous version (+0.2%).
